# dylandreimerink/mimic

Measured on AMD Instinct MI355X. Metric: Mpkts/s (device-resident, one XDP program over 64-1500B batches), higher is better.
Workload: dtype u64; 1 GPU; cfg2: 1M x 64B xdp_md, 36-slot parse+hash DROP/PASS classifier, per-CPU array E=4 S=8; packets_per_gpu=1048576, vcpus_per_gpu=262144, schedule=interleaved, parallelism=dp1, batches_rotated=8, working_set_bytes=713031680, program_slots=36, engine=spread_own, batches_per_launch=8

## Files before the change

include/mimic_amd.h:

```cpp
#ifndef MIMIC_AMD_H
#define MIMIC_AMD_H

#if !defined(__HIPCC_RTC__)
#include <stddef.h>
#include <stdint.h>
#endif

#ifdef __cplusplus
extern "C" {
#endif

#define MIMIC_ABI_VERSION 4

#define MIMIC_EINVAL (-1)
#define MIMIC_ENOMEM (-2)
#define MIMIC_EDEVICE (-3)
#define MIMIC_ENOTSUP (-4)
#define MIMIC_ENOENT (-5)
#define MIMIC_EFAULT (-6)
#define MIMIC_ECANCELED (-7)
#define MIMIC_EDEADLINE (-8)

enum mimic_status {
    MIMIC_OK = 0,
// ... 4 lines not shown
    MIMIC_ERR_MEM_BOUNDS = 5,
    MIMIC_ERR_MEM_NOT_DATASEC = 6,
    MIMIC_ERR_R10_WRITE = 7,
    MIMIC_ERR_HELPER_MAP_PTR = 8,
    MIMIC_ERR_HELPER_KEY = 9,
    MIMIC_ERR_HELPER_VALUE = 10,
    MIMIC_ERR_HELPER_MAP_OP = 11,
    MIMIC_ERR_HELPER_TAILCALL = 12,
    MIMIC_ERR_HELPER_UNIMPLEMENTED = 13,
    MIMIC_ERR_HELPER_CANT_EMULATE = 14,
    MIMIC_ERR_LDABS = 15,
    MIMIC_PANIC_DIV0 = 16,
    MIMIC_PANIC_SHIFT = 17,
    MIMIC_PANIC_BADREG = 18,
    MIMIC_PANIC_CALLX = 19,
    MIMIC_PANIC_PC = 20,
    MIMIC_PANIC_HELPER_NEG = 21,
    MIMIC_ERR_STEP_LIMIT = 22,
    MIMIC_ERR_CALL_DEPTH = 23,
    MIMIC_ERR_ENGINE_HELPER = 24,
    MIMIC_ERR_NO_CPU = 25,
    MIMIC_ERR_CTX_ACCESS = 26,
    MIMIC_PANIC_SLICE = 27,
    MIMIC_ERR_CTX_LOAD = 28,
    MIMIC_ERR_CANCELED = 29,
    MIMIC_ERR_DEADLINE = 30,
    MIMIC_ERR_ENGINE_STATE = 31
};

#define MIMIC_MAP_HASH 1
#define MIMIC_MAP_ARRAY 2
#define MIMIC_MAP_PROG_ARRAY 3
#define MIMIC_MAP_PERCPU_HASH 5
#define MIMIC_MAP_PERCPU_ARRAY 6

#define MIMIC_MAP_F_DATASEC 1u

#define MIMIC_SCHED_CHUNKED 0
#define MIMIC_SCHED_INTERLEAVED 1
#define MIMIC_SCHED_EXPLICIT 2

typedef struct mimic_vm mimic_vm;

typedef struct {
    int32_t vcpus;
    int32_t stack_frame_size;
    int32_t stack_frame_count;
    int32_t max_tail_calls;
    int32_t device;
    int32_t vcpu_begin;
    int32_t vcpu_count;
    int32_t exec_mode;
} mimic_vm_settings;

#define MIMIC_EXEC_DEFAULT 0
#define MIMIC_EXEC_INTERP 1
#define MIMIC_EXEC_JIT 2
#define MIMIC_EXEC_SPREAD 3
#define MIMIC_EXEC_SPREAD_OWN 4

typedef struct {
    const char *name;
    uint32_t type, key_size, value_size, max_entries, flags;
} mimic_map_spec;

typedef struct {
    uint32_t slot;
    uint32_t map_id;
} mimic_reloc;

typedef struct {
    uint32_t n;
    uint32_t schedule;
    uint8_t *pkt_data;
    const uint64_t *pkt_off;
    const uint32_t *pkt_len;
    const uint32_t *headroom;  uint32_t headroom_all;
    const uint32_t *tailroom;  uint32_t tailroom_all;
    const int32_t *ingress_ifindex; int32_t ingress_all;
    const int32_t *rx_queue_index;  int32_t rxq_all;
    const int32_t *egress_ifindex;  int32_t egress_all;
    const int32_t *cpu;
    uint64_t step_budget;
} mimic_xdp_batch;

typedef struct {
    uint64_t *r0;
    uint8_t *status;
    uint32_t *steps;
    int32_t *err_pc;
} mimic_xdp_results;

int mimic_abi_version(void);
const char *mimic_last_error(const mimic_vm *vm);

int mimic_vm_create(const mimic_vm_settings *settings, mimic_vm **out);
void mimic_vm_destroy(mimic_vm *vm);

int mimic_map_create(mimic_vm *vm, const mimic_map_spec *spec, uint32_t *map_id);
int mimic_map_update(mimic_vm *vm, uint32_t map_id, const void *key, const void *value, uint32_t flags, int32_t cpu);
int mimic_map_update_batch(mimic_vm *vm, uint32_t map_id, const void *keys, const void *values, uint32_t n,
                           uint32_t flags, int32_t cpu, int32_t *rc_out);
int mimic_map_lookup(mimic_vm *vm, uint32_t map_id, const void *key, int32_t cpu, uint32_t *addr_out);
int mimic_map_delete(mimic_vm *vm, uint32_t map_id, const void *key);
int mimic_map_keys(mimic_vm *vm, uint32_t map_id, void *out, size_t cap, uint32_t *n_out);
int mimic_map_entries(mimic_vm *vm, uint32_t map_id, void *keys_out, int32_t *slots_out, size_t cap_entries,
                      uint32_t *n_out);
int mimic_map_read_values(mimic_vm *vm, uint32_t map_id, int32_t cpu, void *out, size_t cap);
int mimic_map_reset(mimic_vm *vm, uint32_t map_id, void *hip_stream);
int mimic_map_read_values_range(mimic_vm *vm, uint32_t map_id, int32_t cpu_begin, int32_t cpu_end, void *out,
                                size_t cap);
int mimic_map_sum_u64(mimic_vm *vm, uint32_t map_id, int32_t cpu_begin, int32_t cpu_end, uint64_t *out, size_t cap);
int mimic_map_share(mimic_vm *vm, uint32_t map_id, mimic_vm *owner, uint32_t owner_map_id);
int mimic_map_addr(mimic_vm *vm, uint32_t map_id, uint32_t *addr_out);

int mimic_program_load(mimic_vm *vm, const char *name, const void *insns, uint32_t n_slots,
                       const mimic_reloc *relocs, uint32_t n_relocs, uint32_t *prog_id);
int mimic_program_addr(mimic_vm *vm, uint32_t prog_id, uint32_t *addr_out);

int mimic_mem_read(mimic_vm *vm, uint32_t addr, void *buf, uint32_t len);
int mimic_mem_load(mimic_vm *vm, uint32_t addr, int32_t size, uint64_t *out);
int mimic_stack_addr(mimic_vm *vm, uint32_t *addr_out);

int mimic_run_xdp(mimic_vm *vm, uint32_t prog_id, const mimic_xdp_batch *batch,
                  const mimic_xdp_results *results, void *hip_stream);
int mimic_run_xdp_many(mimic_vm *vm, uint32_t prog_id, const mimic_xdp_batch *batches,
                       const mimic_xdp_results *results, uint32_t k, void *hip_stream);
#define MIMIC_CTX_XDP 0
#define MIMIC_CTX_SKB 1
#define MIMIC_SKB_CUSTOM_SK 1u
#define MIMIC_SKB_CUSTOM_FLOWKEYS 2u
typedef struct {
    uint32_t flags;
    uint32_t sk_bound_dev_if, sk_family, sk_type, sk_protocol, sk_mark, sk_priority;
    uint32_t sk_src_port, sk_dst_port, sk_state;
    int32_t sk_rx_queue_mapping;
    uint8_t sk_ip_len[4];
    uint8_t sk_ip[4][16];
    uint16_t fk_nhoff, fk_thoff, fk_addr_proto;
    uint8_t fk_is_frag, fk_is_first_frag, fk_is_encap, fk_ip_proto;
    uint16_t fk_n_proto, fk_sport, fk_dport;
    uint32_t fk_flags, fk_flow_label;
} mimic_skb_custom;

typedef struct {
    uint32_t n;
    uint32_t schedule;
    uint8_t *pkt_data;
    const uint64_t *pkt_off;
    const uint32_t *pkt_len;
    uint32_t ifindex;
    int32_t pad;
    const int32_t *cpu;
    uint64_t step_budget;
    const mimic_skb_custom *custom;
    uint32_t *rooms_state;
} mimic_skb_batch;

int mimic_run_skb(mimic_vm *vm, uint32_t prog_id, const mimic_skb_batch *batch,
                  const mimic_xdp_results *results, void *hip_stream);
int mimic_skb_release(mimic_vm *vm);

typedef struct mimic_process mimic_process;
typedef struct {
    uint64_t r[11];
    int32_t pc;
    uint32_t prog_id;
    uint64_t steps;
    int32_t status;
    uint32_t exited;
} mimic_process_regs;
int mimic_process_new(mimic_vm *vm, uint32_t prog_id, const void *packet, uint32_t len, uint32_t headroom,
                      uint32_t tailroom, int32_t ingress_ifindex, int32_t rx_queue_index, int32_t egress_ifindex,
                      mimic_process **out);
int mimic_process_new_skb(mimic_vm *vm, uint32_t prog_id, const void *packet, uint32_t len, uint32_t ifindex,
                          mimic_process **out);
// ... 71 lines not shown
```

mimic_amd/_lib.py:

```python
from __future__ import annotations

import ctypes as C
import os

_HERE = os.path.dirname(os.path.abspath(__file__))
LIB_PATH = os.path.join(_HERE, os.path.basename(os.environ.get("MIMIC_LIB", "libmimic_amd.so")))

ABI_VERSION = 4

STATUS_NAMES = [
    "OK", "ERR_PC_OOB", "ERR_UNSUPPORTED_OP", "ERR_MEM_UNRESOLVED", "ERR_MEM_NOT_VMMEM",
    "ERR_MEM_BOUNDS", "ERR_MEM_NOT_DATASEC", "ERR_R10_WRITE", "ERR_HELPER_MAP_PTR",
    "ERR_HELPER_KEY", "ERR_HELPER_VALUE", "ERR_HELPER_MAP_OP", "ERR_HELPER_TAILCALL",
    "ERR_HELPER_UNIMPLEMENTED", "ERR_HELPER_CANT_EMULATE", "ERR_LDABS", "PANIC_DIV0",
    "PANIC_SHIFT", "PANIC_BADREG", "PANIC_CALLX", "PANIC_PC", "PANIC_HELPER_NEG",
    "ERR_STEP_LIMIT", "ERR_CALL_DEPTH", "ERR_ENGINE_HELPER", "ERR_NO_CPU", "ERR_CTX_ACCESS", "PANIC_SLICE",
    "ERR_CTX_LOAD", "ERR_CANCELED", "ERR_DEADLINE", "ERR_ENGINE_STATE",
]
STATUS = {n: i for i, n in enumerate(STATUS_NAMES)}
ECANCELED, EDEADLINE = -7, -8

SCHED_CHUNKED, SCHED_INTERLEAVED, SCHED_EXPLICIT = 0, 1, 2
MAP_F_DATASEC = 1


class VMSettings(C.Structure):
    _fields_ = [("vcpus", C.c_int32), ("stack_frame_size", C.c_int32), ("stack_frame_count", C.c_int32),
                ("max_tail_calls", C.c_int32), ("device", C.c_int32), ("vcpu_begin", C.c_int32),
                ("vcpu_count", C.c_int32), ("exec_mode", C.c_int32)]


class MapSpecC(C.Structure):
    _fields_ = [("name", C.c_char_p), ("type", C.c_uint32), ("key_size", C.c_uint32),
                ("value_size", C.c_uint32), ("max_entries", C.c_uint32), ("flags", C.c_uint32)]


class ProcessRegs(C.Structure):
    _fields_ = [("r", C.c_uint64 * 11), ("pc", C.c_int32), ("prog_id", C.c_uint32), ("steps", C.c_uint64),
                ("status", C.c_int32), ("exited", C.c_uint32)]


class Reloc(C.Structure):
    _fields_ = [("slot", C.c_uint32), ("map_id", C.c_uint32)]


class XDPBatch(C.Structure):
    _fields_ = [("n", C.c_uint32), ("schedule", C.c_uint32), ("pkt_data", C.c_void_p),
                ("pkt_off", C.c_void_p), ("pkt_len", C.c_void_p),
                ("headroom", C.c_void_p), ("headroom_all", C.c_uint32),
                ("tailroom", C.c_void_p), ("tailroom_all", C.c_uint32),
                ("ingress_ifindex", C.c_void_p), ("ingress_all", C.c_int32),
                ("rx_queue_index", C.c_void_p), ("rxq_all", C.c_int32),
                ("egress_ifindex", C.c_void_p), ("egress_all", C.c_int32),
                ("cpu", C.c_void_p), ("step_budget", C.c_uint64)]


class SKBBatch(C.Structure):
    _fields_ = [("n", C.c_uint32), ("schedule", C.c_uint32), ("pkt_data", C.c_void_p),
                ("pkt_off", C.c_void_p), ("pkt_len", C.c_void_p), ("ifindex", C.c_uint32), ("pad", C.c_int32),
                ("cpu", C.c_void_p), ("step_budget", C.c_uint64), ("custom", C.c_void_p), ("rooms_state", C.c_void_p)]


SKB_CUSTOM_SK, SKB_CUSTOM_FLOWKEYS = 1, 2
try:
    import numpy as _np

    SKB_CUSTOM_DTYPE = _np.dtype([
        ("flags", "<u4"), ("sk_bound_dev_if", "<u4"), ("sk_family", "<u4"), ("sk_type", "<u4"), ("sk_protocol", "<u4"),
        ("sk_mark", "<u4"), ("sk_priority", "<u4"), ("sk_src_port", "<u4"), ("sk_dst_port", "<u4"), ("sk_state", "<u4"),
        ("sk_rx_queue_mapping", "<i4"), ("sk_ip_len", "u1", (4,)), ("sk_ip", "u1", (4, 16)),
        ("fk_nhoff", "<u2"), ("fk_thoff", "<u2"), ("fk_addr_proto", "<u2"), ("fk_is_frag", "u1"),
        ("fk_is_first_frag", "u1"), ("fk_is_encap", "u1"), ("fk_ip_proto", "u1"), ("fk_n_proto", "<u2"),
        ("fk_sport", "<u2"), ("fk_dport", "<u2"), ("fk_flags", "<u4"), ("fk_flow_label", "<u4")])
    assert SKB_CUSTOM_DTYPE.itemsize == 136
except ImportError:
    SKB_CUSTOM_DTYPE = None


CTX_XDP, CTX_SKB = 0, 1


class XDPResults(C.Structure):
    _fields_ = [("r0", C.c_void_p), ("status", C.c_void_p), ("steps", C.c_void_p), ("err_pc", C.c_void_p)]


class XDPHostBatch(C.Structure):
    _fields_ = [("n", C.c_uint32), ("schedule", C.c_uint32), ("pkt_data", C.c_void_p),
                ("pkt_off", C.c_void_p), ("pkt_len", C.c_void_p),
                ("headroom_all", C.c_uint32), ("tailroom_all", C.c_uint32),
                ("ingress_all", C.c_int32), ("rxq_all", C.c_int32), ("egress_all", C.c_int32), ("pad", C.c_int32),
                ("cpu", C.c_void_p), ("step_budget", C.c_uint64), ("pkt_out", C.c_void_p),
                ("r0", C.c_void_p), ("status", C.c_void_p)]


EXPORTS = {
    "mimic_abi_version": (C.c_int, []),
    "mimic_last_error": (C.c_char_p, [C.c_void_p]),
    "mimic_vm_create": (C.c_int, [C.POINTER(VMSettings), C.POINTER(C.c_void_p)]),
    "mimic_vm_destroy": (None, [C.c_void_p]),
    "mimic_map_create": (C.c_int, [C.c_void_p, C.POINTER(MapSpecC), C.POINTER(C.c_uint32)]),
    "mimic_map_update": (C.c_int, [C.c_void_p, C.c_uint32, C.c_void_p, C.c_void_p, C.c_uint32, C.c_int32]),
    "mimic_map_lookup": (C.c_int, [C.c_void_p, C.c_uint32, C.c_void_p, C.c_int32, C.POINTER(C.c_uint32)]),
    "mimic_map_update_batch": (C.c_int, [C.c_void_p, C.c_uint32, C.c_void_p, C.c_void_p, C.c_uint32, C.c_uint32,
                                         C.c_int32, C.c_void_p]),
    "mimic_map_delete": (C.c_int, [C.c_void_p, C.c_uint32, C.c_void_p]),
    "mimic_exec_mode": (C.c_int, [C.c_void_p]),
    "mimic_set_spread": (C.c_int, [C.c_void_p, C.c_int32]),
    "mimic_process_new_skb_ctx": (C.c_int, [C.c_void_p, C.c_uint32, C.c_char_p, C.c_uint32, C.c_uint32, C.c_void_p,
                                            C.POINTER(C.c_void_p)]),
    "mimic_run_xdp_host": (C.c_int, [C.c_void_p, C.c_uint32, C.POINTER(XDPHostBatch), C.c_uint32]),
    "mimic_host_register": (C.c_int, [C.c_void_p, C.c_size_t]),
    "mimic_host_unregister": (C.c_int, [C.c_void_p]),
    "mimic_last_exec": (C.c_int, [C.c_void_p]),
    "mimic_jit_source_for": (C.c_long, [C.POINTER(C.c_void_p), C.POINTER(C.c_uint32), C.c_uint32, C.c_char_p,
                                         C.c_size_t]),
    "mimic_jit_check": (C.c_int, [C.c_char_p, C.c_char_p, C.c_size_t, C.POINTER(C.c_size_t)]),
    "mimic_jit_prebuild": (C.c_int, [C.POINTER(C.c_void_p), C.POINTER(C.c_uint32), C.c_uint32]),
    "mimic_map_keys": (C.c_int, [C.c_void_p, C.c_uint32, C.c_void_p, C.c_size_t, C.POINTER(C.c_uint32)]),
    "mimic_map_entries": (C.c_int, [C.c_void_p, C.c_uint32, C.c_void_p, C.c_void_p, C.c_size_t,
                                    C.POINTER(C.c_uint32)]),
    "mimic_map_read_values": (C.c_int, [C.c_void_p, C.c_uint32, C.c_int32, C.c_void_p, C.c_size_t]),
    "mimic_map_reset": (C.c_int, [C.c_void_p, C.c_uint32, C.c_void_p]),
    "mimic_map_read_values_range": (C.c_int, [C.c_void_p, C.c_uint32, C.c_int32, C.c_int32, C.c_void_p, C.c_size_t]),
    "mimic_map_sum_u64": (C.c_int, [C.c_void_p, C.c_uint32, C.c_int32, C.c_int32, C.c_void_p, C.c_size_t]),
    "mimic_map_addr": (C.c_int, [C.c_void_p, C.c_uint32, C.POINTER(C.c_uint32)]),
    "mimic_program_load": (C.c_int, [C.c_void_p, C.c_char_p, C.c_void_p, C.c_uint32, C.POINTER(Reloc),
                                     C.c_uint32, C.POINTER(C.c_uint32)]),
    "mimic_program_addr": (C.c_int, [C.c_void_p, C.c_uint32, C.POINTER(C.c_uint32)]),
    "mimic_mem_read": (C.c_int, [C.c_void_p, C.c_uint32, C.c_void_p, C.c_uint32]),
    "mimic_mem_load": (C.c_int, [C.c_void_p, C.c_uint32, C.c_int32, C.POINTER(C.c_uint64)]),
    "mimic_stack_addr": (C.c_int, [C.c_void_p, C.POINTER(C.c_uint32)]),
    "mimic_run_xdp": (C.c_int, [C.c_void_p, C.c_uint32, C.POINTER(XDPBatch), C.POINTER(XDPResults), C.c_void_p]),
    "mimic_run_xdp_many": (C.c_int, [C.c_void_p, C.c_uint32, C.POINTER(XDPBatch), C.POINTER(XDPResults), C.c_uint32,
                                     C.c_void_p]),
    "mimic_map_share": (C.c_int, [C.c_void_p, C.c_uint32, C.c_void_p, C.c_uint32]),
    "mimic_run_skb": (C.c_int, [C.c_void_p, C.c_uint32, C.POINTER(SKBBatch), C.POINTER(XDPResults), C.c_void_p]),
    "mimic_skb_release": (C.c_int, [C.c_void_p]),
    "mimic_jit_source_for_ctx": (C.c_long, [C.POINTER(C.c_void_p), C.POINTER(C.c_uint32), C.c_uint32, C.c_int32,
                                             C.c_char_p, C.c_size_t]),
    "mimic_jit_source_vc": (C.c_long, [C.POINTER(C.c_void_p), C.POINTER(C.c_uint32), C.c_uint32, C.c_int32,
                                       C.POINTER(C.c_uint32), C.c_uint32, C.c_char_p, C.c_size_t]),
    "mimic_jit_source_spread": (C.c_long, [C.POINTER(C.c_void_p), C.POINTER(C.c_uint32), C.c_uint32,
                                           C.POINTER(C.c_uint32), C.c_uint32, C.POINTER(C.c_uint32), C.c_uint32,
                                           C.c_uint32, C.POINTER(C.c_int32), C.c_char_p, C.c_size_t]),
    "mimic_jit_prebuild_ctx": (C.c_int, [C.POINTER(C.c_void_p), C.POINTER(C.c_uint32), C.c_uint32, C.c_int32]),
    "mimic_jit_cache_source": (C.c_int, [C.c_char_p]),
    "mimic_process_new": (C.c_int, [C.c_void_p, C.c_uint32, C.c_char_p, C.c_uint32, C.c_uint32, C.c_uint32,
                                    C.c_int32, C.c_int32, C.c_int32, C.POINTER(C.c_void_p)]),
    "mimic_process_new_skb": (C.c_int, [C.c_void_p, C.c_uint32, C.c_char_p, C.c_uint32, C.c_uint32, C.c_void_p]),
    "mimic_process_set_cpu": (C.c_int, [C.c_void_p, C.c_int32]),
    "mimic_process_step": (C.c_int, [C.c_void_p, C.c_uint32, C.c_void_p]),
    "mimic_process_run": (C.c_int, [C.c_void_p, C.c_uint64, C.c_void_p]),
    "mimic_process_packet": (C.c_int, [C.c_void_p, C.c_void_p, C.c_size_t]),
    "mimic_process_free": (None, [C.c_void_p]),
    "mimic_jit_code": (C.c_int, [C.c_char_p, C.c_void_p, C.c_size_t, C.POINTER(C.c_size_t)]),
    "mimic_sync": (C.c_int, [C.c_void_p, C.c_void_p]),
    "mimic_ctx_new": (C.c_int, [C.c_uint64, C.POINTER(C.c_void_p)]),
    "mimic_ctx_cancel": (None, [C.c_void_p]),
    "mimic_ctx_err": (C.c_int, [C.c_void_p]),
    "mimic_ctx_pinned": (C.c_int, [C.c_void_p]),
    "mimic_ctx_free": (None, [C.c_void_p]),
    "mimic_run_xdp_ctx": (C.c_int, [C.c_void_p, C.c_uint32, C.POINTER(XDPBatch), C.POINTER(XDPResults), C.c_void_p,
                                    C.c_void_p, C.c_void_p]),
    "mimic_run_skb_ctx": (C.c_int, [C.c_void_p, C.c_uint32, C.POINTER(SKBBatch), C.POINTER(XDPResults), C.c_void_p,
                                    C.c_void_p, C.c_void_p]),
    "mimic_process_run_ctx": (C.c_int, [C.c_void_p, C.c_uint64, C.c_void_p, C.POINTER(ProcessRegs)]),
    "mimic_process_run_many": (C.c_int, [C.c_void_p, C.c_uint32, C.c_void_p, C.c_void_p, C.POINTER(ProcessRegs)]),
    "mimic_process_free_many": (None, [C.c_void_p, C.c_uint32]),
    "mimic_run_xdp_host_ctx": (C.c_int, [C.c_void_p, C.c_uint32, C.POINTER(XDPHostBatch), C.c_uint32, C.c_void_p]),
    "mimic_run_xdp_host_ctx_pp": (C.c_int, [C.c_void_p, C.c_uint32, C.POINTER(XDPHostBatch), C.c_uint32, C.c_void_p]),
    "mimic_last_steps": (C.c_int, [C.c_void_p, C.POINTER(C.c_uint64)]),
}

_lib = None


def load() -> C.CDLL:
    global _lib
    if _lib is not None:
        return _lib
    if not os.path.exists(LIB_PATH):
        raise ImportError(f"{LIB_PATH} is missing: run __graft_entry__.build() (hipcc --offload-arch=gfx950)")
    try:
        import torch
    except ImportError:
        pass
    lib = C.CDLL(LIB_PATH)
    for name, (res, args) in EXPORTS.items():
        fn = getattr(lib, name)
        fn.restype = res
        fn.argtypes = args
    if lib.mimic_abi_version() != ABI_VERSION:
        raise ImportError("libmimic_amd.so ABI version mismatch")
    _lib = lib
    return lib
```

mimic_amd/csrc/engine.cpp:

```cpp
#include <hip/hip_runtime.h>

#include <algorithm>
#include <atomic>
#include <cstdarg>
#include <cstdlib>
#include <cstdio>
#include <cstring>
#include <map>
#include <string>
#include <chrono>
#include <condition_variable>
#include <memory>
#include <mutex>
#include <thread>
#include <unordered_map>
#include <vector>

#include "../../include/mimic_amd.h"
#include "blkcache.h"
#include "layout.h"
#include "hashmap.h"
#include "jit.h"
#include "skb.h"

// ... 500 lines not shown
    vm->d_segs = nullptr;
    vm->d_maps = nullptr;
    HIP_OK(vm, hipMalloc(&vm->d_insns, all.size() * sizeof(DInsn)));
    HIP_OK(vm, hipMalloc(&vm->d_progs, dp.size() * sizeof(DProg)));
    HIP_OK(vm, hipMalloc(&vm->d_segs, sg.size() * sizeof(Seg)));
    HIP_OK(vm, hipMalloc(&vm->d_maps, dm.size() * sizeof(DMap)));
    HIP_OK(vm, hipMemcpy(vm->d_insns, all.data(), all.size() * sizeof(DInsn), hipMemcpyHostToDevice));
    HIP_OK(vm, hipMemcpy(vm->d_progs, dp.data(), dp.size() * sizeof(DProg), hipMemcpyHostToDevice));
    HIP_OK(vm, hipMemcpy(vm->d_segs, sg.data(), sg.size() * sizeof(Seg), hipMemcpyHostToDevice));
    HIP_OK(vm, hipMemcpy(vm->d_maps, dm.data(), dm.size() * sizeof(DMap), hipMemcpyHostToDevice));
    vm->tables_dirty = false;
    return 0;
}

struct HostRef {
    int kind;
    uint64_t dev_off;
    uint32_t off, limit;
};

static HostRef host_resolve(const mimic_vm *vm, uint32_t a) {
    HostRef R{0, 0, 0, 0};
    for (const Seg &g : vm->segs) {
        if (a < g.lo || a > g.hi) continue;
        uint32_t off = a - g.lo;
        switch (g.kind) {
        case SEG_PLAIN: R = {1, g.dev_off, off, g.size}; break;
        case SEG_ARRAY_OBJ: R = {g.datasec ? 1 : 3, g.dev_off, off, g.size}; break;
        case SEG_MAP_OBJ: case SEG_PROG: R = {2, 0, 0, 0}; break;
        case SEG_PERCPU_ARRAY: {
            uint32_t c = off / g.period, r = off - c * g.period;
            uint64_t base = g.dev_off + (uint64_t)c * g.dev_stride;
            if (r <= 8) R = {g.datasec ? 1 : 3, base, r, g.size};
            else R = {1, base, r - 9, g.size};
            break;
        }
        case SEG_PERCPU_VALUES: {
            uint32_t c = off / g.period, r = off - c * g.period;
            R = {1, g.dev_off + (uint64_t)c * g.dev_stride, r, g.size};
            break;
        }
        }
        return R;
    }
    return R;
}

static int decode_program(const uint8_t *raw, uint32_t n_slots, std::vector<DInsn> &out, std::string *err) {
    out.assign(n_slots, DInsn{0, 0, 0});
    for (uint32_t i = 0; i < n_slots; i++) {
        const uint8_t *b = raw + 8ull * i;
        uint32_t op = b[0], dst = b[1] & 0xf, src = b[1] >> 4;
        uint16_t off = (uint16_t)(b[2] | (b[3] << 8));
        int32_t imm;
        memcpy(&imm, b + 4, 4);
        DInsn d{};
        d.w = op | (dst << 8) | (src << 12) | ((uint32_t)off << 16);
        d.k = (uint64_t)(int64_t)imm;
        if (op == 0x18) {
            if (i + 1 >= n_slots) {
                *err = "64bit immediate is missing second half";
                return -1;
            }
            const uint8_t *c = b + 8;
            if (c[0] | c[1] | c[2] | c[3]) {
                *err = "64bit immediate has non-zero fields";
                return -1;
            }
            uint32_t hi;
            memcpy(&hi, c + 4, 4);
            d.k = ((uint64_t)hi << 32) | (uint32_t)imm;
            out[i] = d;
            out[++i] = DInsn{0, 0, 0};
            continue;
        }
        out[i] = d;
    }
    return 0;
}

extern "C" {

int mimic_abi_version(void) { return MIMIC_ABI_VERSION; }

const char *mimic_last_error(const mimic_vm *vm) { return vm ? vm->err.c_str() : "null vm"; }

int mimic_vm_create(const mimic_vm_settings *settings, mimic_vm **out) {
    if (!settings || !out) return MIMIC_EINVAL;
    if (settings->vcpus <= 0) return MIMIC_EINVAL;
    mimic_vm *vm = new mimic_vm();
    vm->s = *settings;
    if (vm->s.stack_frame_size <= 0) vm->s.stack_frame_size = 256;
    if (vm->s.stack_frame_count <= 0) vm->s.stack_frame_count = 8;
    if (vm->s.vcpu_count <= 0) {
        vm->s.vcpu_begin = 0;
        vm->s.vcpu_count = vm->s.vcpus;
    }
    if (vm->s.vcpu_begin < 0 || vm->s.vcpu_begin + vm->s.vcpu_count > vm->s.vcpus) {
        delete vm;
        return MIMIC_EINVAL;
    }
    if (stack_size(vm) % 8 != 0 || stack_size(vm) > (1u << 20)) {
        delete vm;
        return MIMIC_EINVAL;
    }
    vm->exec_mode = settings->exec_mode;
    if (vm->exec_mode == MIMIC_EXEC_DEFAULT) {
        const char *e = getenv("MIMIC_EXEC");
        vm->exec_mode = (e && !strcmp(e, "interp")) ? MIMIC_EXEC_INTERP : MIMIC_EXEC_JIT;
    }
    if (const char *pj = getenv("MIMIC_PROC_JIT")) vm->proc_jit_after = *pj ? atoll(pj) : 32;
    if (vm->exec_mode != MIMIC_EXEC_INTERP && vm->exec_mode != MIMIC_EXEC_JIT) {
        delete vm;
        return MIMIC_EINVAL;
    }
    if (hipSetDevice(vm->s.device) != hipSuccess || hipStreamCreateWithFlags(&vm->stream, hipStreamNonBlocking) != hipSuccess) {
        delete vm;
        return MIMIC_EDEVICE;
    }
    *out = vm;
    return 0;
}

void mimic_vm_destroy(mimic_vm *vm) {
    if (!vm) return;
    hipSetDevice(vm->s.device);
    hipDeviceSynchronize();
    for (auto &m : vm->maps) {
        if (!m.share) continue;
        auto &mem = m.share->members;
        if (!mem.empty() && mem[0].vm == vm) m.share->owner_gone = true;
        for (size_t k = 0; k < mem.size(); k++)
            if (mem[k].vm == vm) {
                if (k == 0) hipDeviceSynchronize();
                mem.erase(mem.begin() + (long)k);
                break;
            }
        m.share.reset();
    }
    vm->blk.drain([](Blk &b) {
        hipFree(b.dev);
        if (b.host) hipHostFree(b.host);
    });
    hipFree(vm->arena);
    hipFree(vm->d_insns);
    hipFree(vm->d_progs);
    hipFree(vm->d_segs);
    hipFree(vm->d_maps);
    hipFree(vm->priv);
    hipFree(vm->d_sched_start);
    hipFree(vm->d_sched_pkts);
    hipFree(vm->d_lane_steps);
    hipFree(vm->d_spread_bad);
    hipFree(vm->d_spread_part);
    hipFree(vm->d_cancel_pp);
    hipFree(vm->d_defer);
    hipFree(vm->d_defer_any);
    hipFree(vm->d_kp);
    if (vm->h_kp) hipHostFree(vm->h_kp);
    for (auto &sl : vm->slot) {
        hipFree(sl.buf);
        hipFree(sl.off);
        hipFree(sl.len);
        hipFree(sl.r0);
        hipFree(sl.st);
        for (hipEvent_t e : {sl.e_in, sl.e_k, sl.e_out})
// ... 775 lines not shown
    g.lo = p.addr;
    g.hi = p.addr + 8;
    g.kind = SEG_PROG;
    g.id = (uint32_t)vm->progs.size();
    vm->segs.push_back(g);
    vm->progs.push_back(std::move(p));
    vm->tables_dirty = true;
    *prog_id = g.id;
    return 0;
}

int mimic_program_addr(mimic_vm *vm, uint32_t prog_id, uint32_t *addr_out) {
    if (!vm || prog_id >= vm->progs.size()) return MIMIC_EINVAL;
    *addr_out = vm->progs[prog_id].addr;
    return 0;
}

int mimic_stack_addr(mimic_vm *vm, uint32_t *addr_out) {
    if (!vm) return MIMIC_EINVAL;
    *addr_out = vm->next_addr;
    return 0;
}

int mimic_mem_read(mimic_vm *vm, uint32_t addr, void *buf, uint32_t len) {
    if (!vm) return MIMIC_EINVAL;
    hipSetDevice(vm->s.device);
    HostRef R = host_resolve(vm, addr);
    if (R.kind == 0) return fail(vm, MIMIC_EFAULT, "memory controller can't resolve address 0x%x", addr);
    if (R.kind == 2) return fail(vm, MIMIC_EFAULT, "not vm memory 0x%x", addr);
    if (R.kind == 3) return fail(vm, MIMIC_EFAULT, "Can't access non-data-section array map directly");
    if ((uint64_t)R.off + len > R.limit) return fail(vm, MIMIC_EFAULT, "out of bounds");
    if (int rc = flush_host(vm)) return rc;
    if (vm->last_stream) HIP_OK(vm, hipStreamSynchronize(vm->last_stream));
    HIP_OK(vm, hipMemcpy(buf, vm->arena + R.dev_off + R.off, len, hipMemcpyDeviceToHost));
    return 0;
}

int mimic_mem_load(mimic_vm *vm, uint32_t addr, int32_t size, uint64_t *out) {
    if (size != 1 && size != 2 && size != 4 && size != 8) return MIMIC_EINVAL;
    uint64_t v = 0;
    int rc = mimic_mem_read(vm, addr, &v, (uint32_t)size);
    if (rc) return rc;
    *out = v;
    return 0;
}

struct SkbRun {
    uint32_t ifindex;
    const mimic_skb_custom *custom;
    const uint64_t *pre_drv = nullptr, *pre_prefix = nullptr, *pre_base = nullptr;
    uint32_t *rooms_state = nullptr;
};
struct StepRun {
    StepState *state;
    uint8_t *priv;
    uint64_t priv_bytes;
    uint64_t budget;
    SkbRec *skb_rec = nullptr;
    const uint64_t *skb_prefix = nullptr, *skb_base = nullptr;
    const mimic_skb_custom *skb_custom = nullptr;
    uint32_t gen = 0;
    const uint8_t *img = nullptr;
    uint8_t *img_dst = nullptr;
    uint32_t img_n = 0;
    bool jit = false;
    int32_t cpu = 0;
};

struct CtxRun {
    mimic_ctx *all;
    mimic_ctx *const *per_packet;
    const uint32_t *const *dev_pp = nullptr;
};
struct ManyRun {
    const mimic_xdp_batch *b;
    const mimic_xdp_results *r;
    uint32_t k;
    bool used;
};
static int run_xdp_impl(mimic_vm *vm, uint32_t prog_id, const mimic_xdp_batch *b, const mimic_xdp_results *res,
                        hipStream_t st_in, uint64_t shift, const SkbRun *skb = nullptr, const StepRun *step = nullptr,
                        const CtxRun *cx = nullptr, ManyRun *mr = nullptr);

int mimic_run_xdp(mimic_vm *vm, uint32_t prog_id, const mimic_xdp_batch *b, const mimic_xdp_results *res,
                  void *hip_stream) {
    return run_xdp_impl(vm, prog_id, b, res, (hipStream_t)hip_stream, 0);
}

int mimic_run_xdp_many(mimic_vm *vm, uint32_t prog_id, const mimic_xdp_batch *b, const mimic_xdp_results *res, uint32_t k,
                       void *hip_stream) {
    if (!vm || (k && (!b || !res))) return MIMIC_EINVAL;
    hipStream_t st = (hipStream_t)hip_stream;
    auto same = [&](const mimic_xdp_batch &x, const mimic_xdp_batch &y) {
        return x.n == y.n && x.schedule == y.schedule && x.schedule != MIMIC_SCHED_EXPLICIT && !x.headroom && !y.headroom &&
               !x.tailroom && !y.tailroom && !x.ingress_ifindex && !y.ingress_ifindex && !x.rx_queue_index &&
               !y.rx_queue_index && !x.egress_ifindex && !y.egress_ifindex && x.headroom_all == y.headroom_all &&
               x.tailroom_all == y.tailroom_all && x.ingress_all == y.ingress_all && x.rxq_all == y.rxq_all &&
               x.egress_all == y.egress_all && x.step_budget == y.step_budget;
    };
    for (uint32_t a = 0; a < k;) {
        uint32_t e = a + 1;
        while (e < k && e - a < MIMIC_MANY_MAX && same(b[a], b[e])) e++;
        ManyRun mr{b + a, res + a, e - a, false};
        int rc = run_xdp_impl(vm, prog_id, b + a, res + a, st, 0, nullptr, nullptr, nullptr, e - a > 1 ? &mr : nullptr);
        if (rc) return rc;
        if (!mr.used)
            for (uint32_t q = a + 1; q < e; q++)
                if ((rc = run_xdp_impl(vm, prog_id, b + q, res + q, st, 0))) return rc;
        a = e;
    }
    return 0;
}

int mimic_run_xdp_ctx(mimic_vm *vm, uint32_t prog_id, const mimic_xdp_batch *b, const mimic_xdp_results *res,
                      void *hip_stream, mimic_ctx *ctx, mimic_ctx *const *ctx_per_packet) {
    const CtxRun cx{ctx, ctx_per_packet};
    return run_xdp_impl(vm, prog_id, b, res, (hipStream_t)hip_stream, 0, nullptr, nullptr, &cx);
}

static int run_skb_impl(mimic_vm *vm, uint32_t prog_id, const mimic_skb_batch *sb, const mimic_xdp_results *res,
                        void *hip_stream, const CtxRun *cx);

int mimic_run_skb(mimic_vm *vm, uint32_t prog_id, const mimic_skb_batch *sb, const mimic_xdp_results *res,
                  void *hip_stream) {
    return run_skb_impl(vm, prog_id, sb, res, hip_stream, nullptr);
}

int mimic_run_skb_ctx(mimic_vm *vm, uint32_t prog_id, const mimic_skb_batch *sb, const mimic_xdp_results *res,
                      void *hip_stream, mimic_ctx *ctx, mimic_ctx *const *ctx_per_packet) {
    const CtxRun cx{ctx, ctx_per_packet};
    return run_skb_impl(vm, prog_id, sb, res, hip_stream, &cx);
}

static int run_skb_impl(mimic_vm *vm, uint32_t prog_id, const mimic_skb_batch *sb, const mimic_xdp_results *res,
                        void *hip_stream, const CtxRun *cx) {
    if (!vm || !sb || !res) return MIMIC_EINVAL;
    mimic_xdp_batch b{};
    b.n = sb->n;
    b.schedule = sb->schedule;
    b.pkt_data = sb->pkt_data;
    b.pkt_off = sb->pkt_off;
    b.pkt_len = sb->pkt_len;
    b.cpu = sb->cpu;
    b.step_budget = sb->step_budget;
    SkbRun r{sb->ifindex, sb->custom};
    r.rooms_state = sb->rooms_state;
    return run_xdp_impl(vm, prog_id, &b, res, (hipStream_t)hip_stream, 0, &r, nullptr, cx);
}

int mimic_skb_release(mimic_vm *vm) {
    if (!vm) return MIMIC_EINVAL;
    hipSetDevice(vm->s.device);
    if (vm->skb_stream) {
        if (!vm->skb_ev) HIP_OK(vm, hipEventCreateWithFlags(&vm->skb_ev, hipEventDisableTiming));
        HIP_OK(vm, hipEventRecord(vm->skb_ev, vm->skb_stream));
        vm->skb_stream = nullptr;
        vm->skb_release_pending = true;
    }
    vm->skb_leaked = false;
    return 0;
}

static int skb_settle(mimic_vm *vm) {
    if (vm->skb_release_pending) HIP_OK(vm, hipEventSynchronize(vm->skb_ev));
    vm->skb_release_pending = false;
    return 0;
}

struct SkbInto {
    SkbRec *rec;
    uint64_t *prefix;
};
static int skb_ensure(mimic_vm *vm, uint32_t n, hipStream_t st);
static int skb_prepare(mimic_vm *vm, const mimic_xdp_batch *b, hipStream_t st, const SkbInto *into = nullptr,
                       uint32_t *rooms_state = nullptr) {
// ... 105 lines not shown

static int spread_build_own(mimic_vm *vm) {
    if (vm->spread_own_state) return 0;
    vm->spread_own_state = -1;
    SpreadReq req;
    req.own = true;
    for (size_t s = 0; s < vm->h_all.size(); s++) {
        const DInsn &x = vm->h_all[s];
        const uint32_t mh = AUX_MAPHINT(x.aux);
        if (AUX_H(x.aux) != H_LDIMM || !mh || mh > vm->maps.size()) continue;
        const HostMap &hm = vm->maps[mh - 1];
        const DMap dm = to_dmap(hm);
        if (hm.family != FAM_PERCPU_ARRAY || (dm.dev_off & 7) || (dm.dev_stride & 7)) continue;
        req.slot_map[(uint32_t)s] = mh - 1;
        req.shape[mh - 1] = {hm.max_entries * hm.value_size, hm.value_size};
    }
    if (req.slot_map.empty()) return 0;
    uint32_t row = 0;
    for (auto &kv : req.shape) row = std::max(row, kv.second.first);
    if (!row) return 0;
    req.lds_rows = std::min<uint32_t>(256u, 32768u / row);
    if (req.lds_rows < 2) return 0;
    JitInfo info{};
    const std::string src = mimic_jit_source(vm->h_dp, vm->h_all, CTX_XDP, &info, nullptr, false, &req);
    if (!info.spread || !info.spread_own) return 0;
    std::string log;
    if (mimic_jit_compile(vm->s.device, src, &vm->jit_fn_spread_own, &log))
        return fail(vm, MIMIC_EDEVICE, "JIT build failed (owned spread kernel): %s", log.c_str());
    vm->jit_info_spread_own = info;
    vm->spread_own_rows = req.lds_rows;
    vm->spread_own_state = 1;
    return 0;
}

static int priv_ensure(mimic_vm *vm, uint32_t q_per_lane, uint32_t lanes, hipStream_t st) {
    const uint32_t stride = std::max(lanes, vm->priv_lanes);
    const uint64_t need = (uint64_t)q_per_lane * stride * 8;
    if (vm->priv && need <= vm->priv_bytes) return 0;
    hipStreamSynchronize(st);
    hipFree(vm->priv);
    vm->priv = nullptr;
    HIP_OK(vm, hipMalloc(&vm->priv, std::max<uint64_t>(need, 8)));
    vm->priv_bytes = std::max<uint64_t>(need, 8);
    vm->priv_lanes = stride;
    return 0;
}

static int spread_check(mimic_vm *vm) {
    if (vm->comb_used) {
        for (const HostMap &m : vm->maps) {
            if (!is_hash(m)) continue;
            uint64_t rb, fo, co;
            ht_offsets(m, &rb, &fo, &co);
            uint32_t f = 0;
            HIP_OK(vm, hipMemcpy(&f, vm->arena + m.ht_dev_off + co + offsetof(HashCtl, comb_fault), 4, hipMemcpyDeviceToHost));
            if (f) return fail(vm, MIMIC_EDEVICE, "map '%s': a block combiner or chunk refill of freelist reservations gave up (engine fault)",
                               m.name.c_str());
        }
    }
    if (!vm->spread_used || !vm->d_spread_bad) return 0;
    uint32_t f = 0;
    HIP_OK(vm, hipMemcpy(&f, vm->d_spread_bad, 4, hipMemcpyDeviceToHost));
    if (f) return fail(vm, MIMIC_EDEVICE, "a spread launch reached per-CPU map memory outside a fused increment");
    return 0;
}

static std::vector<std::pair<uint32_t, uint32_t>> vc_slots_of(const mimic_vm *vm) {
    std::vector<std::pair<uint32_t, uint32_t>> vc;
    for (size_t s = 0; s < vm->h_all.size(); s++) {
        const DInsn &x = vm->h_all[s];
        const uint32_t mh = AUX_MAPHINT(x.aux);
        if (AUX_H(x.aux) != H_LDIMM || !mh || mh > vm->maps.size()) continue;
        const HostMap &hm = vm->maps[mh - 1];
        if (vc_row_ok(hm.family, hm.max_entries, hm.value_size)) vc.push_back({(uint32_t)s, hm.max_entries * hm.value_size});
    }
    return vc;
}

static int run_xdp_impl(mimic_vm *vm, uint32_t prog_id, const mimic_xdp_batch *b, const mimic_xdp_results *res,
                        hipStream_t st_in, uint64_t first_index, const SkbRun *skb, const StepRun *step,
                        const CtxRun *cx, ManyRun *mr) {
    if (!vm || !b || !res) return MIMIC_EINVAL;
    if (prog_id >= vm->progs.size()) return fail(vm, MIMIC_EINVAL, "no program with id '%u' is loaded", prog_id);
    if (b->n > 0 && (!b->pkt_data || !b->pkt_off || !b->pkt_len)) return fail(vm, MIMIC_EINVAL, "missing packet arrays");
    if (cx && cx->all && cx->per_packet) return fail(vm, MIMIC_EINVAL, "one context for the batch or one per packet, not both");
    if (cx && cx->all && !cx->all->pinned) return fail(vm, MIMIC_EDEVICE, "the context was made without a device");
    if (cx && cx->per_packet)
        for (uint32_t i = 0; i < b->n; i++)
            if (cx->per_packet[i] && !cx->per_packet[i]->pinned)
                return fail(vm, MIMIC_EDEVICE, "packet %u: the context was made without a device", i);
    if (!skb) {
        const int rc = skb_settle(vm);
        if (rc) return rc;
    }
    if (!skb && vm->skb_leaked)
        return fail(vm, MIMIC_ENOTSUP, "xdp_md batches after sk_buff batches are not supported (mimic_skb_release first)");
    const uint32_t ctx = skb ? CTX_SKB : CTX_XDP;
    hipSetDevice(vm->s.device);
    int rc = upload_tables(vm);
    if (!rc) rc = flush_host(vm);
    if (rc) return rc;
    hipStream_t st = st_in ? st_in : vm->stream;
    const uint32_t cpu_lanes = step ? 1u : (uint32_t)vm->s.vcpu_count;
    const bool proc_jit = step && step->jit;
    bool extra = false;
    if (!step && b->schedule == MIMIC_SCHED_EXPLICIT && b->cpu)
        for (uint32_t i = 0; i < b->n && !extra; i++) extra = b->cpu[i] == -1 || b->cpu[i] == vm->s.vcpus;
    const uint32_t lanes = cpu_lanes + (extra ? 2u : 0u);
    const uint32_t S = stack_size(vm);
    const PrivPlan pp = priv_plan(vm);
    const uint32_t xdp_q = pp.xdp_q, frame_q = pp.frame_q, key_q = pp.key_q, q_per_lane = pp.q_per_lane;
    const uint32_t plan = (lanes + 255) & ~255u;
    if (step) {
        if (step->priv_bytes < (uint64_t)q_per_lane * 8) return fail(vm, MIMIC_EINVAL, "process private memory too small");
    } else {
        rc = priv_ensure(vm, q_per_lane, plan, st);
        if (rc) return rc;
    }
    if (lanes > vm->lane_steps_cap) {
        hipStreamSynchronize(st);
        hipFree(vm->d_lane_steps);
        vm->d_lane_steps = nullptr;
        HIP_OK(vm, hipMalloc(&vm->d_lane_steps, (uint64_t)plan * sizeof(uint64_t)));
        vm->lane_steps_cap = plan;
    }
    KParams kp{};
    kp.insns = vm->d_insns;
    kp.progs = vm->d_progs;
    kp.segs = vm->d_segs;
    kp.maps = vm->d_maps;
    kp.arena = vm->arena;
    kp.nprogs = (uint32_t)vm->progs.size();
    kp.nsegs = (uint32_t)vm->segs.size();
    kp.nmaps = (uint32_t)vm->maps.size();
    kp.entry_prog = prog_id;
    kp.static_next = vm->next_addr;
    kp.stack_size = S;
    kp.frame_size = (uint32_t)vm->s.stack_frame_size;
    uint32_t shift = 3;
    while (S > 512 && ((S - 512 + (1u << shift) - 1) >> shift) > 64) shift++;
    kp.chunk_shift = shift;
    kp.max_tail_calls = (uint32_t)std::max(0, vm->s.max_tail_calls);
    kp.total_vcpus = (uint32_t)vm->s.vcpus;
    kp.vcpu_begin = proc_jit ? (uint32_t)step->cpu : (uint32_t)vm->s.vcpu_begin;
    kp.lanes = lanes;
    kp.cpu_lanes = cpu_lanes;
    kp.priv_lanes = step ? 1u : vm->priv_lanes;
    kp.priv = step ? step->priv : vm->priv;
    kp.priv_xdp_q = xdp_q;
    kp.priv_frame_q = frame_q;
    kp.priv_key_q = key_q;
    kp.budget = step ? step->budget : (b->step_budget ? b->step_budget : MIMIC_DEFAULT_BUDGET);
    kp.step = step ? step->state : nullptr;
    kp.step_gen = step ? step->gen : 0u;
    if (step) {
        kp.step_img = step->img;
        kp.step_dst = step->img_dst;
        kp.step_img_n = step->img_n;
        kp.step_ins_n = (uint32_t)std::min<size_t>(vm->h_all.size(), 2048);
    }
    kp.n = b->n;
    kp.sched = b->schedule;
    kp.pkt_data = b->pkt_data;
    kp.pkt_off = b->pkt_off;
    kp.pkt_len = b->pkt_len;
    kp.headroom_arr = b->headroom;
    kp.tailroom_arr = b->tailroom;
    kp.ingress_arr = b->ingress_ifindex;
    kp.rxq_arr = b->rx_queue_index;
    kp.egress_arr = b->egress_ifindex;
    kp.headroom = b->headroom_all;
    kp.tailroom = b->tailroom_all;
    kp.ingress = b->ingress_all;
    kp.rxq = b->rxq_all;
    kp.egress = b->egress_all;
    kp.r0 = res->r0;
    kp.status = res->status;
    kp.steps = res->steps;
    kp.err_pc = res->err_pc;
    kp.lane_steps = vm->d_lane_steps;
    if (cx && cx->all) {
        kp.cancel = cx->all->dword;
        kp.cancel_any = 1;
    } else if (cx && cx->dev_pp && b->n) {
        kp.cancel_pp = cx->dev_pp;
        kp.cancel_any = 1;
    } else if (cx && cx->per_packet && b->n) {
        std::vector<const uint32_t *> w(b->n);
        bool any = false;
        for (uint32_t i = 0; i < b->n; i++) {
            w[i] = cx->per_packet[i] ? cx->per_packet[i]->dword : nullptr;
            any |= w[i] != nullptr;
        }
        if (any) {
            if (vm->cancel_pp_stream) hipStreamSynchronize(vm->cancel_pp_stream);
            hipStreamSynchronize(st);
            vm->cancel_pp_stream = st;
            if (b->n > vm->cancel_pp_cap) {
                hipFree(vm->d_cancel_pp);
                vm->d_cancel_pp = nullptr;
                HIP_OK(vm, hipMalloc(&vm->d_cancel_pp, (size_t)b->n * sizeof(void *)));
                vm->cancel_pp_cap = b->n;
            }
            HIP_OK(vm, hipMemcpy(vm->d_cancel_pp, w.data(), (size_t)b->n * sizeof(void *), hipMemcpyHostToDevice));
            kp.cancel_pp = vm->d_cancel_pp;
            kp.cancel_any = 1;
        }
    }
    switch (b->schedule) {
    case MIMIC_SCHED_CHUNKED:
        kp.per_lane = lanes ? (uint32_t)(((uint64_t)b->n + lanes - 1) / lanes) : 0;
        break;
    case MIMIC_SCHED_INTERLEAVED:
        kp.sched_shift = lanes ? (uint32_t)(first_index % lanes) : 0;
        kp.per_lane = lanes ? (uint32_t)(((uint64_t)b->n + kp.sched_shift + lanes - 1) / lanes) : 0;
        break;
    case MIMIC_SCHED_EXPLICIT: {
        if (!b->cpu && b->n) return fail(vm, MIMIC_EINVAL, "explicit schedule needs cpu[]");
        std::vector<uint32_t> start(lanes + 1, 0), pk(b->n);
        std::vector<uint32_t> lane_of(b->n);
        for (uint32_t i = 0; i < b->n; i++) {
            const int32_t id = b->cpu[i];
            int64_t c = (int64_t)id - vm->s.vcpu_begin;
            if (id == -1) c = cpu_lanes;
            else if (id == vm->s.vcpus) c = cpu_lanes + 1;
            else if (c < 0 || c >= (int64_t)cpu_lanes)
                return fail(vm, MIMIC_EINVAL, "packet %u: cpu %d not on this engine", i, id);
            lane_of[i] = (uint32_t)c;
            start[c + 1]++;
        }
        uint32_t mx = 0;
        for (uint32_t c = 0; c < lanes; c++) {
            mx = std::max(mx, start[c + 1]);
            start[c + 1] += start[c];
        }
        std::vector<uint32_t> fill(start.begin(), start.end() - 1);
        for (uint32_t i = 0; i < b->n; i++) pk[fill[lane_of[i]]++] = i;
        hipStreamSynchronize(st);
        if (start.size() > vm->sched_cap_start) {
            hipFree(vm->d_sched_start);
            vm->d_sched_start = nullptr;
            HIP_OK(vm, hipMalloc(&vm->d_sched_start, start.size() * 4));
            vm->sched_cap_start = start.size();
        }
        if (pk.size() > vm->sched_cap_pkts || !vm->d_sched_pkts) {
            hipFree(vm->d_sched_pkts);
            vm->d_sched_pkts = nullptr;
            HIP_OK(vm, hipMalloc(&vm->d_sched_pkts, std::max<size_t>(pk.size(), 1) * 4));
// ... 116 lines not shown
            }
            kp.spread_part = vm->d_spread_part;
        }
    }
    if (skb && step && step->skb_rec) {
        kp.ctx_kind = CTX_SKB;
        kp.skb_ifindex = skb->ifindex;
        kp.skb_rec = step->skb_rec;
        kp.skb_prefix = step->skb_prefix;
        kp.skb_base = step->skb_base;
        kp.skb_custom = step->skb_custom;
    } else if (skb && skb->pre_drv) {
        rc = skb_ensure(vm, b->n, st);
        if (rc) return rc;
        kp.ctx_kind = CTX_SKB;
        kp.skb_ifindex = skb->ifindex;
        kp.skb_rec = vm->d_skb_rec;
        kp.skb_drv = skb->pre_drv;
        kp.skb_prefix = skb->pre_prefix;
        kp.skb_base = skb->pre_base;
        kp.skb_custom = skb->custom;
        vm->skb_stream = st;
    } else if (skb) {
        rc = skb_prepare(vm, b, st, nullptr, skb->rooms_state);
        if (rc) return rc;
        kp.skb_rooms_state = skb->rooms_state;
        kp.ctx_kind = CTX_SKB;
        kp.skb_ifindex = skb->ifindex;
        kp.skb_rec = vm->d_skb_rec;
        kp.skb_drv = vm->d_skb_drv;
        kp.skb_prefix = vm->d_skb_prefix;
        kp.skb_base = vm->d_skb_state + 1;
        kp.skb_custom = skb->custom;
    }
    kp.hash_pop_only = vm->prog_deletes ? 0u : 1u;
    kp.hash_ro = (vm->prog_deletes || vm->prog_updates) ? 0u : 1u;
    for (auto &m : vm->maps) {
        if (!is_hash(m)) continue;
        if (m.share) {
            if ((rc = share_check(vm, m))) return rc;
            for (auto &mb : m.share->members) {
                mimic_vm *o = (mimic_vm *)mb.vm;
                if (o != vm && o->host_dirty && (rc = flush_host(o))) return fail(vm, rc, "shared map: %s", o->err.c_str());
            }
            share_stale(m);
        }
        const DMap dm = to_dmap(m);
        if (vm->prog_deletes && m.pop_dirty) {
            if (mimic_launch_hash_normalize(vm->arena, &dm, st))
                return fail(vm, MIMIC_EDEVICE, "launch: %s", hipGetErrorString(hipGetLastError()));
            m.pop_dirty = false;
        }
        if (!vm->prog_deletes) m.pop_dirty = true;
        if (vm->prog_deletes) m.may_tomb = true;
        if (m.mir && (vm->prog_updates || vm->prog_deletes || m.may_tomb)) m.mir->valid = false;
        if (!m.may_tomb) continue;
        if (mimic_launch_hash_rebuild(vm->arena, &dm, 0, st))
            return fail(vm, MIMIC_EDEVICE, "launch: %s", hipGetErrorString(hipGetLastError()));
    }
    vm->last_exec = jit ? (own ? MIMIC_EXEC_SPREAD_OWN : spread ? MIMIC_EXEC_SPREAD : MIMIC_EXEC_JIT) : MIMIC_EXEC_INTERP;
    if (jit && ji.defer) {
        if (lanes > vm->defer_cap || !vm->d_defer_any) {
            hipStreamSynchronize(st);
            hipFree(vm->d_defer);
            vm->d_defer = nullptr;
            HIP_OK(vm, hipMalloc(&vm->d_defer, (uint64_t)plan * sizeof(DeferRec)));
            HIP_OK(vm, hipMemset(vm->d_defer, 0, (uint64_t)plan * sizeof(DeferRec)));
            vm->defer_cap = plan;
            if (!vm->d_defer_any) {
                HIP_OK(vm, hipMalloc(&vm->d_defer_any, 64));
                HIP_OK(vm, hipMemset(vm->d_defer_any, 0, 64));
            }
        }
        if (++vm->defer_epoch == 0) vm->defer_epoch = 1;
        kp.defer = vm->d_defer;
        kp.defer_any = vm->d_defer_any;
        kp.defer_epoch = vm->defer_epoch;
    }
    if (jit && ji.hash_combine) vm->comb_used = true;
    if (mr) {
        mr->used = jit && own && !ji.defer && mr->k >= 1 && mr->k <= MIMIC_MANY_MAX;
        if (mr->used) {
            kp.many_n = mr->k;
            for (uint32_t q = 0; q < mr->k; q++)
                kp.many[q] = BatchRef{mr->b[q].pkt_data, mr->b[q].pkt_off, mr->b[q].pkt_len, mr->r[q].r0, mr->r[q].status,
                                      mr->r[q].steps, mr->r[q].err_pc, 0};
        }
    }
    if (jit) {
        if (mimic_jit_launch(jfn, &kp, st))
            return fail(vm, MIMIC_EDEVICE, "launch: %s", hipGetErrorString(hipGetLastError()));
        if (ji.defer && mimic_launch_xdp_resume(&kp, st))
            return fail(vm, MIMIC_EDEVICE, "launch: %s", hipGetErrorString(hipGetLastError()));
    } else if (step) {
        if (mimic_launch_xdp(&kp, nullptr, st))
            return fail(vm, MIMIC_EDEVICE, "launch: %s", hipGetErrorString(hipGetLastError()));
    } else {
        const KParams *dkp = nullptr;
        const int slot = kp_slot(vm, kp, st, &dkp);
        if (slot < 0) return slot;
        if (mimic_launch_xdp(&kp, dkp, st))
            return fail(vm, MIMIC_EDEVICE, "launch: %s", hipGetErrorString(hipGetLastError()));
        HIP_OK(vm, hipEventRecord(vm->kp_ev[slot], st));
        vm->kp_used[slot] = true;
    }
    if (jit && ji.hash_chunk) {
        for (const HostMap &m : vm->maps) {
            if (!m.chunk) continue;
            const DMap dm = to_dmap(m);
            if (mimic_launch_hash_compact(vm->arena, &dm, st))
                return fail(vm, MIMIC_EDEVICE, "launch: %s", hipGetErrorString(hipGetLastError()));
        }
    }
    if (jit && kp.spread_part) {
        const DMap dm = to_dmap(vm->maps[ji.spread_map]);
        if (mimic_launch_spread_reduce(kp.spread_part, kp.lanes / 256u, kp.cpu_lanes, ji.spread_roww, ji.spread_n,
                                       vm->arena + dm.dev_off + (uint64_t)kp.vcpu_begin * dm.dev_stride, dm.dev_stride, st))
            return fail(vm, MIMIC_EDEVICE, "launch: %s", hipGetErrorString(hipGetLastError()));
    }
    if (kp.cancel_any) {
        auto mark = [&](mimic_ctx *c) -> int {
            std::lock_guard<std::mutex> lk(c->mu);
            std::vector<hipEvent_t> keep;
            for (hipEvent_t e : c->uses) {
                if (hipEventQuery(e) == hipSuccess) hipEventDestroy(e);
                else keep.push_back(e);
            }
            c->uses.swap(keep);
            hipEvent_t ev = nullptr;
            HIP_OK(vm, hipEventCreateWithFlags(&ev, hipEventDisableTiming));
            HIP_OK(vm, hipEventRecord(ev, st));
            c->uses.push_back(ev);
            return 0;
        };
        if (cx->all) {
            if ((rc = mark(cx->all))) return rc;
        } else {
            std::vector<mimic_ctx *> u;
            for (uint32_t i = 0; i < b->n; i++)
                if (cx->per_packet[i]) u.push_back(cx->per_packet[i]);
            std::sort(u.begin(), u.end());
            u.erase(std::unique(u.begin(), u.end()), u.end());
            for (mimic_ctx *c : u)
                if ((rc = mark(c))) return rc;
        }
    }
    vm->last_lanes = run_lanes;
    vm->last_stream = st;
    return 0;
}

}

namespace {
constexpr size_t PD_LEN = 8, PD_SKB = 64;
constexpr size_t PD_PKT = (PD_SKB + sizeof(SkbRec) + 24 + sizeof(mimic_skb_custom) + 63) & ~(size_t)63;
constexpr size_t PH_RES = (sizeof(StepState) + 63) & ~(size_t)63;
constexpr size_t PH_R0 = PH_RES, PH_ST = PH_RES + 8, PH_STEPS = PH_RES + 16, PH_EPC = PH_RES + 20, PH_WORD = PH_RES + 24;
constexpr size_t PH_IMG = PH_RES + 64;
}

struct mimic_process {
    mimic_vm *vm = nullptr;
    uint32_t prog = 0;
    uint32_t H = 0, T = 0, len = 0;
    int32_t ingress = 0, rxq = 0, egress = 0;
    uint8_t *d_pkt = nullptr;
    uint8_t *d_skbmem = nullptr;
    StepState *hs = nullptr;
// ... 888 lines not shown
```

mimic_amd/csrc/interp.hip:

```cpp
#include <hip/hip_runtime.h>
#include <stdint.h>
#include <algorithm>
#include <cstdlib>

#include "runtime.h"
static_assert(sizeof(Lane) <= sizeof(((StepState *)0)->lane), "StepState::lane too small");
static __device__ void step_save(const KParams &kp, const Lane &L, const uint64_t *RB, int st, int32_t pc, uint32_t steps,
                                 uint32_t prog) {
    StepState *S = kp.step;
    for (int q = 0; q < 11; q++) S->r[q] = RB[q * 64];
    __builtin_memcpy(S->lane, &L, sizeof(Lane));
    S->pc = pc;
    S->prog = prog;
    S->steps = steps;
    S->status = st;
    S->started = 1;
    S->finished = st != MIMIC_ERR_STEP_LIMIT;
}

#define WAVES_PER_BLOCK 4

static __device__ __noinline__ void step_warm(const KParams &kp, uint32_t t, uint32_t nt) {
    const DProg last = kp.progs[kp.nprogs - 1];
    const uint64_t spans[5][2] = {{(uint64_t)(uintptr_t)kp.insns, (uint64_t)(last.base + last.n) * sizeof(DInsn)},
                                  {(uint64_t)(uintptr_t)kp.segs, (uint64_t)kp.nsegs * sizeof(Seg)},
                                  {(uint64_t)(uintptr_t)kp.maps, (uint64_t)kp.nmaps * sizeof(DMap)},
                                  {(uint64_t)(uintptr_t)kp.progs, (uint64_t)kp.nprogs * sizeof(DProg)},
                                  {(uint64_t)(uintptr_t)kp.pkt_data, 512}};
    uint32_t n = 0;
    for (int k = 0; k < 5; k++) {
        const uint64_t lines = (spans[k][1] + 63) / 64;
        for (uint64_t q = t; q < lines && q < 4096; q += nt) n += *(const volatile uint32_t *)(spans[k][0] + q * 64);
    }
    if (t == 0) n += *(const volatile uint32_t *)kp.pkt_off + *(const volatile uint32_t *)kp.pkt_len;
    (void)n;
}
#define NREGS 11
#define KEY_DONE 0xffffffffu

enum { MODE_BATCH = 0, MODE_STEP = 1, MODE_RESUME = 2 };
template <int MODE>
static __device__ __forceinline__ void xdp_body(const KParams *__restrict__ kpp, uint32_t goff = 0) {
    const KParams &kp = *kpp;
    StepState *const STP = MODE == MODE_STEP ? kp.step : nullptr;
    __shared__ uint64_t sreg[WAVES_PER_BLOCK][NREGS][64];
    uint64_t *const RB = &sreg[threadIdx.x >> 6][0][threadIdx.x & 63];
#define REG(r) RB[(r) * 64]

    const uint32_t g = goff + blockIdx.x * blockDim.x + threadIdx.x;
    const DeferRec *DR = nullptr;
    uint32_t j0 = 0;
    if (MODE == MODE_RESUME) {
        if (*kp.defer_any != kp.defer_epoch) return;
        if (g < kp.lanes && kp.defer[g].flag == kp.defer_epoch) {
            DR = kp.defer + g;
            j0 = DR->j;
        }
        if (__ballot(DR != nullptr) == 0) return;
    }
    const bool lane_valid = g < kp.lanes && (MODE != MODE_RESUME || DR);
    extern __shared__ DInsn step_ins_[];
    if (MODE == MODE_STEP) {
        if (kp.step_img) {
            typedef uint32_t u32x4 __attribute__((ext_vector_type(4)));
            const uint32_t nq = kp.step_img_n >> 4;
            for (uint32_t q = threadIdx.x; q < nq; q += blockDim.x)
                ((u32x4 *)kp.step_dst)[q] = ((const u32x4 *)kp.step_img)[q];
            for (uint32_t b = (nq << 4) + threadIdx.x; b < kp.step_img_n; b += blockDim.x) kp.step_dst[b] = kp.step_img[b];
        }
        for (uint32_t q = threadIdx.x; q < kp.step_ins_n; q += blockDim.x) step_ins_[q] = kp.insns[q];
        __syncthreads();
        if (threadIdx.x >= 64) step_warm(kp, threadIdx.x - 64, blockDim.x - 64);
    }
    Lane L;
    L.lane = g;
    L.cpu = STP ? STP->cpu : lane_cpu(kp, g);

    uint32_t ex_begin = 0, ex_count = 0;
    if (lane_valid && kp.sched == SCHED_EXPLICIT) {
        ex_begin = kp.sched_start[g];
        ex_count = kp.sched_start[g + 1] - ex_begin;
    }
    uint64_t lane_steps = MODE == MODE_RESUME && DR ? DR->lane_steps : 0;
    const DProg entry = cget(kp.progs, kp.entry_prog);
    const uint32_t P = kp.static_next + kp.stack_size + 1;

    for (uint32_t j = 0; j < kp.per_lane; j++) {
        uint32_t i = 0xffffffffu;
        if (lane_valid && (MODE != MODE_RESUME || j >= j0)) {
            if (kp.sched == SCHED_CHUNKED) {
                uint64_t ii = (uint64_t)g * kp.per_lane + j;
                if (ii < kp.n) i = (uint32_t)ii;
            } else if (kp.sched == SCHED_INTERLEAVED) {
                uint64_t ii = (uint64_t)j * kp.lanes + (g >= kp.sched_shift ? g - kp.sched_shift : g + kp.lanes - kp.sched_shift);
                if (ii < kp.n) i = (uint32_t)ii;
            } else if (j < ex_count) {
                i = kp.sched_pkts[ex_begin + j];
            }
        }

#pragma unroll
        for (int q = 0; q < NREGS; q++) REG(q) = 0;
        uint32_t pn = entry.n, pbase = entry.base;
        uint32_t cur_prog = kp.entry_prog;
        uint32_t key = KEY_DONE;
        uint32_t steps = 0;
        L.sm0 = 0;
        L.sm1 = 0;
        L.xdp_dirty = 0;
        L.t_n = 0;
        L.t_lo = 0;
        L.t_ptr = nullptr;
        L.nframes = 0;
        L.tailcalls = 0;
        L.M = 0;
        L.pkt = nullptr;
        L.rec = nullptr;
        L.pa = P;
        L.ka = 0;
#define TERM(st_, epc_)                                                \
        do {                                                           \
            if (kp.r0) kp.r0[i] = REG(0);                              \
            if (kp.status) kp.status[i] = (uint8_t)(st_);              \
            if (kp.steps) kp.steps[i] = steps;                         \
            if (kp.err_pc) kp.err_pc[i] = (int32_t)(epc_);             \
            lane_steps += steps;                                       \
            key = KEY_DONE;                                            \
            if (STP) step_save(kp, L, RB, (st_), (epc_), steps, cur_prog); \
        } while (0)
        bool resumed = false, foreign = false;
        if (i != 0xffffffffu && STP && STP->gen != kp.step_gen) {
            foreign = true;
            if (kp.r0) kp.r0[i] = 0;
            if (kp.status) kp.status[i] = (uint8_t)MIMIC_ERR_ENGINE_STATE;
            if (kp.steps) kp.steps[i] = 0;
            if (kp.err_pc) kp.err_pc[i] = -1;
        } else if (i != 0xffffffffu && STP && STP->started) {
            const StepState *S = STP;
#pragma unroll
            for (int q = 0; q < NREGS; q++) REG(q) = S->r[q];
            __builtin_memcpy(&L, S->lane, sizeof(Lane));
            L.cpu = S->cpu;
            steps = S->steps;
            cur_prog = S->prog;
            const DProg cp = kp.progs[cur_prog];
            pn = cp.n;
            pbase = cp.base;
            resumed = true;
            if (S->pc < 0) {
                steps++;
                TERM(MIMIC_PANIC_PC, S->pc);
            } else {
                key = pbase + (uint32_t)S->pc;
            }
        }
        const bool resume_here = MODE == MODE_RESUME && i != 0xffffffffu && j == j0;
        if (resumed || foreign) {
        } else if (i != 0xffffffffu && kp.ctx_kind == CTX_SKB) {
            uint64_t r1 = 0;
            const int ls = skb_load(kp, L, i, r1, resume_here);
            REG(10) = kp.static_next + kp.frame_size;
            if (ls) {
                TERM(ls, -1);
            } else {
                REG(1) = r1;
                key = pbase;
                if (pn == 0) {
                    steps = 1;
                    TERM(MIMIC_ERR_PC_OOB, 0);
                }
            }
        } else if (i != 0xffffffffu) {
            const uint32_t H = kp.headroom_arr ? kp.headroom_arr[i] : kp.headroom;
            const uint32_t T = kp.tailroom_arr ? kp.tailroom_arr[i] : kp.tailroom;
            const uint32_t len = kp.pkt_len[i];
            L.pkt = kp.pkt_data + kp.pkt_off[i];
            L.M = H + len + T;
            if (!resume_here) {
                for (uint32_t b = 0; b < H; b++) L.pkt[b] = 0;
                for (uint32_t b = 0; b < T; b++) L.pkt[H + len + b] = 0;
            }
            L.data = P + H;
            L.data_end = P + H + len;
            L.ingress = (uint32_t)(kp.ingress_arr ? kp.ingress_arr[i] : kp.ingress);
            L.rxq = (uint32_t)(kp.rxq_arr ? kp.rxq_arr[i] : kp.rxq);
            L.egress = (uint32_t)(kp.egress_arr ? kp.egress_arr[i] : kp.egress);
            REG(1) = P + L.M + 1;
            REG(10) = kp.static_next + kp.frame_size;
            key = pbase;
            if (pn == 0) {
                steps = 1;
                TERM(MIMIC_ERR_PC_OOB, 0);
            }
        }

        if (resume_here) {
#pragma unroll
            for (int q = 0; q < NREGS; q++) REG(q) = DR->r[q];
            L.sm0 = DR->sm0;
            L.sm1 = DR->sm1;
            L.xdp_dirty = DR->xdp_dirty;
            L.nframes = DR->nframes;
            L.tailcalls = DR->tailcalls;
            steps = DR->steps;
            cur_prog = DR->prog;
            const DProg cp = kp.progs[cur_prog];
            pn = cp.n;
            pbase = cp.base;
            key = pbase + (uint32_t)DR->pc;
            resumed = true;
        }

        if (MODE != MODE_STEP && kp.cancel_any && !resumed && key != KEY_DONE) {
            const uint32_t cz = ctx_done(kp, i);
            if (cz) TERM(MIMIC_ERR_CANCELED - 1 + (int)cz, (int32_t)(key - pbase));
        }
        uint64_t wsteps = resumed ? steps : 0;
        uint32_t cand = KEY_DONE;
        for (;;) {
            if (MODE != MODE_STEP && kp.cancel_any && (wsteps & 4095u) == 4095u && key != KEY_DONE) {
                const uint32_t cz = ctx_done(kp, i);
                if (cz) TERM(MIMIC_ERR_CANCELED - 1 + (int)cz, (int32_t)(key - pbase));
            }
            uint32_t kw;
            uint64_t act;
            if (MODE == MODE_STEP) {
                kw = (uint32_t)__builtin_amdgcn_readfirstlane((int)key);
                if (kw == KEY_DONE) break;
                act = 1;
            } else {
                const uint64_t live = __ballot(key != KEY_DONE);
                if (live == 0) break;
                if (cand != KEY_DONE && (__ballot(key != cand) & live) == 0) kw = cand;
                else kw = wave_min(key);
                kw = (uint32_t)__builtin_amdgcn_readfirstlane((int)kw);
                act = __ballot(key == kw);
            }
            const DInsn in = MODE == MODE_STEP && kw < kp.step_ins_n ? step_ins_[kw] : cget(kp.insns, kw);
            const uint64_t wbefore = wsteps++;
            if (key == kw) {
                const uint32_t pc = kw - pbase;
                if (wbefore >= kp.budget && (uint64_t)steps == kp.budget) {
                    TERM(MIMIC_ERR_STEP_LIMIT, pc);
                } else {
                    steps++;
                    const uint32_t aux = in.aux;
                    const uint32_t op = in.w & 0xff;
                    const uint32_t dst = (in.w >> 8) & 0xf, src = (in.w >> 12) & 0xf;
                    const int32_t off = (int16_t)(in.w >> 16);
                    const uint64_t k = in.k;
                    int st = 0;
                    int jmp = 0;
                    uint32_t nk = 0;
                    switch (AUX_H(aux)) {
                    case H_NOP:
                        break;
                    case H_ALU64: {
                        const uint64_t d = REG(dst);
                        const uint64_t x = (aux & AUX_X) ? REG(src) : k;
// ... 549 lines not shown
```

mimic_amd/csrc/jit.cpp:

```cpp
#include <hip/hip_runtime.h>
#include <hip/hiprtc.h>

#include <algorithm>
#include <cinttypes>
#include <cstdarg>
#include <cstdio>
#include <cstring>
#include <cstdlib>
#include <unistd.h>
#include <map>
#include <mutex>
#include <set>
#include <string>
#include <vector>

#include "../../include/mimic_amd.h"
#include "layout.h"
#include "jit.h"

namespace {

#include "jit_headers.inc"

struct Emitter {
// ... 213 lines not shown
            hash_combine = combine_knob && writes && !deletes && cold_inline && fast_paths;
            if (hash_combine) E.line("#define MIMIC_HASH_COMBINE 1");
            hash_chunk = hash_combine && !proc && hchunk_knob > 0;
            if (hash_chunk) E.line("#define MIMIC_HASH_CHUNK 1\n#define MIMIC_HCHUNK %uu", (uint32_t)hchunk_knob);
        }
        E.line("#include \"runtime.h\"");
        if (spread_on) {
            E.line("#define SPREAD_MAP %uu        // the per-CPU array the fused increments go to", spread_map);
            E.line("#define SPREAD_N %uu          // counter width (bytes)", spread_n);
            E.line("#define SPREAD_ROWW %uu       // counters per vCPU row (E * S / N)", spread_row / spread_n);
            E.line("#define SPREAD_ROWS %uu       // LDS table rows (0: agent-scope atomics into the map)", spread_req->lds_rows);
            E.line("#define SPREAD_PPB %uu        // packets per block", spread_req->ppb);
            E.line("typedef %s spread_t;", spread_n == 8 ? "unsigned long long" : "uint32_t");
            E.line("#if SPREAD_ROWS");
            E.line("#define spread_add(k_) __hip_atomic_fetch_add(&sacc_[srow_ * SPREAD_ROWW + (uint32_t)(ga_ - L.t_lo) / SPREAD_N], (spread_t)(k_), __ATOMIC_RELAXED, __HIP_MEMORY_SCOPE_WORKGROUP)");
            E.line("#else");
            E.line("#define spread_add(k_) __hip_atomic_fetch_add((GAS spread_t *)(L.t_ptr + (uint32_t)(ga_ - L.t_lo)), (spread_t)(k_), __ATOMIC_RELAXED, __HIP_MEMORY_SCOPE_AGENT)");
            E.line("#endif");
        }
        if (proc) {
            E.line("#define PGID_ kp.entry_prog");
            E.line("#define TERM(s_, pc_) do { st_ = (int)(s_); epc_ = (int32_t)(pc_); pg_ = PGID_; goto L_term; } while (0)");
        } else {
            E.line("#define TERM(s_, pc_) do { st_ = (int)(s_); epc_ = (int32_t)(pc_); goto L_term; } while (0)");
        }
        E.line("#define SPILL() do { sp_.L = L; sp_.r[0] = r0; sp_.r[1] = r1; sp_.r[2] = r2; sp_.r[3] = r3; sp_.r[4] = r4; "
               "sp_.r[5] = r5; sp_.r[6] = r6; } while (0)");
        E.line("#define FILL() do { r0 = sp_.r[0]; r1 = sp_.r[1]; r2 = sp_.r[2]; r3 = sp_.r[3]; r4 = sp_.r[4]; r5 = sp_.r[5]; "
               "L.sm0 = sp_.L.sm0; L.sm1 = sp_.L.sm1; L.xdp_dirty = sp_.L.xdp_dirty; L.t_lo = sp_.L.t_lo; L.t_n = sp_.L.t_n; "
               "L.t_ptr = sp_.L.t_ptr; } while (0)");
        E.line("#define COLD_CALL(call_, pc_) do { VC_FLUSH(); SPILL(); call_; FILL(); if (sp_.st) TERM(sp_.st, pc_); } while (0)");
        E.line("#define DFR(pc_, prog_) do { dr_->pc = (int32_t)(pc_); dr_->prog = (prog_); dr_->steps = steps - 1u; goto L_defer; } while (0)");
        if (vc_on && vc_lds)
            E.line("#define VC_FLUSH() do { if (vcd_) { lvc_writeback(vcp_, vcb_, lvt_); vcd_ = 0u; } vcv_ = 0u; } while (0)");
        else if (vc_on)
            E.line("#define VC_FLUSH() do { if (vcd_) { vc_writeback(vcp_, vcb_, vc0_, vc1_, vc2_, vc3_); vcd_ = 0u; } vcv_ = 0u; } while (0)");
        else
            E.line("#define VC_FLUSH() do { } while (0)");
        const int wv = proc ? 0 : waves > 0 ? waves : (cold_inline ? 4 : 0);
        E.line("extern \"C\" __global__ __launch_bounds__(256) %svoid mimic_jit_kernel(const KParams kp_arg_) {",
               wv > 0 ? ("__attribute__((amdgpu_waves_per_eu(" + std::to_string(wv) + "))) ").c_str() : "");
        E.line("  (void)kp_arg_;   // the first (only) kernel argument: at offset 0 of the kernarg segment");
        E.line("  const KParams __attribute__((address_space(4))) *kp4_ = (const KParams __attribute__((address_space(4))) *)__builtin_amdgcn_kernarg_segment_ptr();");
        E.line("  asm volatile(\"\" : \"+s\"(kp4_));");
        E.line("  const KParams *kpp = (const KParams *)kp4_;");
        E.line("  const KParams &kp = *kpp;");
        E.line("  const uint32_t g = blockIdx.x * blockDim.x + threadIdx.x;");
        if (hash_chunk) E.line("  h_chunk_init(%s);   // (its waves: those the early return below keeps)", spread_on ? "0xffffffffu" : "kp.lanes");
        if (hash_combine) E.line("  h_comb_init();   // before any thread of the block can leave");
        if (!spread_on) E.line("  if (g >= kp.lanes) return;");
        skb_lds = ctx == CTX_SKB && fast_paths && skb_fields && skb_lds_knob;
        if (skb_lds) E.line("  __shared__ uint64_t srec_[%uu * 256u];", kSrecQ);
        E.line("  Lane L;");
        E.line("  Spill sp_;");
        if (census) {
            E.line("  uint32_t coldn_ = 0;");
            E.line("#define COLD_CALL_K(k_, call_, pc_) do { coldn_ += 1u << (k_); COLD_CALL(call_, pc_); } while (0)");
        }
        E.line("  L.lane = g;");
        if (spread_own) {
            E.line("  const uint32_t oP_ = kp.per_lane, oQ_ = kp.own_q, oS_ = oP_ / oQ_, oR_ = 256u / oS_;");
            E.line("  const uint32_t orow_ = threadIdx.x %% oR_, oj_ = threadIdx.x / oR_, olane_ = blockIdx.x * oR_ + orow_;");
            E.line("  const uint32_t osh_ = olane_ >= kp.sched_shift ? olane_ - kp.sched_shift : olane_ + kp.cpu_lanes - kp.sched_shift;");
            E.line("#define OWN_IDX_I(k_) ((oj_ < oS_ && olane_ < kp.cpu_lanes && (uint64_t)(oj_ + (k_) * oS_) * kp.cpu_lanes + osh_ < kp.n) ? (uint32_t)((uint64_t)(oj_ + (k_) * oS_) * kp.cpu_lanes + osh_) : NO_PKT)");
            E.line("#define OWN_IDX_C(k_) ((threadIdx.x + 256u * (k_) < oR_ * oP_ && (uint64_t)blockIdx.x * oR_ * oP_ + threadIdx.x + 256u * (k_) < kp.n) ? (uint32_t)((uint64_t)blockIdx.x * oR_ * oP_ + threadIdx.x + 256u * (k_)) : NO_PKT)");
            E.line("#define OWN_IDX(k_) (kp.sched == SCHED_CHUNKED ? OWN_IDX_C(k_) : OWN_IDX_I(k_))");
            E.line("  const uint32_t oi_ = OWN_IDX(0u);");
            E.line("  const bool ochk_ = kp.sched == SCHED_CHUNKED;");
            E.line("  const uint64_t ostr64_ = ochk_ ? 256ull : (uint64_t)oS_ * kp.cpu_lanes;");
            E.line("  const uint64_t oend_ = (uint64_t)blockIdx.x * oR_ * oP_ + (uint32_t)(oR_ * oP_);");
            E.line("  uint32_t ofl_ = __builtin_amdgcn_readfirstlane((kp.headroom_arr || kp.tailroom_arr || kp.ingress_arr || kp.rxq_arr || kp.egress_arr ? 1u : 0u) | (kp.headroom | kp.tailroom ? 2u : 0u));");
            E.line("  uint32_t ocpu_ = kp.vcpu_begin + olane_, oep_ = kp.entry_prog, or10_ = kp.static_next + kp.frame_size;");
            E.line("  uint32_t ostr_ = ostr64_ < 0xffffffffull ? (uint32_t)ostr64_ : 0xffffffffu;");
            E.line("  uint32_t olim_ = ochk_ && oend_ < kp.n ? (uint32_t)oend_ : kp.n;");
            E.line("  asm volatile(\"\" : \"+s\"(ostr_), \"+s\"(olim_), \"+s\"(ofl_), \"+s\"(oep_), \"+s\"(or10_));");
            E.line("  asm volatile(\"\" : \"+v\"(ocpu_));");
            E.line("  uint32_t oin_ = (uint32_t)kp.ingress, orx_ = (uint32_t)kp.rxq, oeg_ = (uint32_t)kp.egress;");
            E.line("  asm volatile(\"\" : \"+s\"(oin_), \"+s\"(orx_), \"+s\"(oeg_));");
            E.line("%s", kOwnHoist);
            E.line("  const DMap SM_ = cget(kp.maps, SPREAD_MAP);");
            E.line("  __shared__ spread_t sacc_[SPREAD_ROWS * SPREAD_ROWW];");
            E.line("  for (uint32_t w_ = threadIdx.x; w_ < SPREAD_ROWS * SPREAD_ROWW; w_ += 256u) sacc_[w_] = 0;");
            E.line("  __shared__ BatchRef obr_[MIMIC_MANY_MAX];");
            E.line("  if (threadIdx.x < (kp.many_n ? kp.many_n : 1u)) obr_[threadIdx.x] = kp.many_n ? cget(kp.many, threadIdx.x) : BatchRef{kp.pkt_data, kp.pkt_off, kp.pkt_len, kp.r0, kp.status, kp.steps, kp.err_pc, 0};");
            E.line("  __syncthreads();");
            E.line("  uint32_t srow_ = orow_, sbase_ = 0;");
            E.line("  const bool ofw_ = threadIdx.x < oR_ * SPREAD_ROWW && blockIdx.x * oR_ + threadIdx.x / SPREAD_ROWW < kp.cpu_lanes;");
            E.line("  GAS spread_t *const ofd_ = (GAS spread_t *)(kp.arena + SM_.dev_off + (size_t)(kp.vcpu_begin + blockIdx.x * oR_ + threadIdx.x / SPREAD_ROWW) * SM_.dev_stride) + threadIdx.x %% SPREAD_ROWW;");
            E.line("  const spread_t ofv_ = ofw_ ? *ofd_ : (spread_t)0;");
        } else if (spread_on) {
            E.line("  const uint32_t blo_ = blockIdx.x * SPREAD_PPB, bhi_ = blo_ + SPREAD_PPB < kp.n ? blo_ + SPREAD_PPB : kp.n;");
            E.line("  const uint32_t lam0_ = spread_lane(kp, blo_);");
            E.line("  const DMap SM_ = cget(kp.maps, SPREAD_MAP);");
            E.line("#if SPREAD_ROWS");
            E.line("  __shared__ spread_t sacc_[SPREAD_ROWS * SPREAD_ROWW];");
            E.line("  for (uint32_t w_ = threadIdx.x; w_ < SPREAD_ROWS * SPREAD_ROWW; w_ += 256u) sacc_[w_] = 0;");
            E.line("  __syncthreads();");
            E.line("#endif");
            E.line("  uint32_t srow_ = 0, sbase_ = 0;");
            E.line("  const uint32_t lstep_ = 256u %% kp.cpu_lanes;");
            E.line("  uint32_t lam_ = spread_lane(kp, blo_ + threadIdx.x);");
        } else {
            E.line("  L.cpu = lane_cpu(kp, g);");
        }
        if (vc_on) {
            if (vc_lds) {
                E.line("  __shared__ uint32_t lvc_[(%uu / 4u + 2u) * 256u];", vc_rb);
                E.line("  uint32_t *const lvt_ = lvc_ + threadIdx.x;");
                E.line("  constexpr uint32_t vcb_ = %uu;   // the row's bytes", vc_rb);
                E.line("  uint32_t vcv_ = 0u, vcd_ = 0u, vclo_ = 0u; uint8_t *vcp_ = nullptr;");
                E.line("  { const uint32_t mh_ = AUX_MAPHINT(cget(kp.insns, %uu).aux);", vc_slot);
                E.line("    if (mh_) lvc_open(kp, cget(kp.maps, mh_ - 1u), L.cpu, vcb_, vcp_, vclo_, vcv_, lvt_); }");
            } else {
                E.line("  uint64_t vc0_ = 0, vc1_ = 0, vc2_ = 0, vc3_ = 0; uint32_t vcv_ = 0u, vcd_ = 0u, vclo_ = 0u, vcb_ = 0u; uint8_t *vcp_ = nullptr;");
                E.line("  { const uint32_t mh_ = AUX_MAPHINT(cget(kp.insns, %uu).aux);", vc_slot);
                E.line("    if (mh_) vc_open(kp, cget(kp.maps, mh_ - 1u), L.cpu, vcp_, vclo_, vcb_, vcv_, vc0_, vc1_, vc2_, vc3_); }");
            }
        }
        E.line("  uint32_t ex_begin = 0, ex_count = 0;");
        E.line("  if (kp.sched == SCHED_EXPLICIT) { ex_begin = *gp(kp.sched_start + g); ex_count = *gp(kp.sched_start + g + 1) - ex_begin; }");
        E.line("  uint64_t lane_steps = 0;");
        E.line("  const uint32_t P = kp.static_next + kp.stack_size + 1;");
        if (ctx == CTX_SKB) E.line("  const uint32_t SK_ = P;   // the sk_buff entry (skb.h)");
        E.line("  uint32_t ga_ = 0;   // the address of the current memory access");
        if (ret_dispatch && any_local) E.line("  uint32_t ret_ = 0;   // the slot a popped frame returns to (R<p>_)");
        for (auto &f : fwd_store) E.line("  uint32_t fwd%u_%u_ = 0;   // value of the stack store at P%u slot %u", f.first, f.second, f.first, f.second);
        for (auto &u : spec_use)
            E.line("  %s sp%u_%u_ = 0;   // packet load of P%u slot %u, issued early", u.second == 8 ? "uint64_t" : "uint32_t",
                   u.first.first, u.first.second, u.first.first, u.first.second);
        if (!spec_use.empty()) E.line("  uint32_t spv_ = 1;   // 0 once a store through R10 left the stack: early values void");
        const bool pf = ctx == CTX_XDP && prefetch;
        if (!spec_use.empty() && !spread_on) analyze_xpf();
        lpf_on = pf && xpf.on && lpf_knob && !xpf_knob && !spread_on && !vc_lds && !lds_stack_on && !defer_mode &&
                 !hash_combine && lpf_safe();
        if (!lpf_on && !xpf_knob) xpf.on = false;
        if (spread_own) {
            if (pf) E.line("  uint64_t noff_ = 0, poff_ = 0; uint32_t nlen_ = 0, plen_ = 0;");
            E.line("  const uint32_t nb_ = kp.many_n ? kp.many_n : 1u;");
            E.line("  bool bpre_ = false;   // this batch's first descriptor came with the previous batch's last packet");
            E.line("  for (uint32_t bt_ = 0; bt_ < nb_; bt_++) {");
            E.line("  const BatchRef br_ = kp.many_n ? cget(kp.many, bt_) : BatchRef{kp.pkt_data, kp.pkt_off, kp.pkt_len, kp.r0, kp.status, kp.steps, kp.err_pc, 0};");
        }
        if (lpf_on) {
            const uint32_t D = kLpfD, XW = xpf.words;
            E.line("  // lane prefetch: packets 0..%u of the lane, descriptors + P%u slot %u window (data + %u, %u words)", D - 1,
                   xpf.prog, xpf.hp, (uint32_t)xpf.off, XW);
            E.line("  __shared__ uint64_t lpfo_[%uu * 256u];", D);
            E.line("  __shared__ uint32_t lpfl_[%uu * 256u];", D);
            E.line("  __shared__ uint64_t lpfw_[%uu * 256u];", D * XW);
            E.line("  uint32_t lpf_n_ = 0u, xc_ok_ = 0u;");
            E.line("  if (kp.entry_prog == %uu && !kp.headroom_arr && !kp.tailroom_arr && kp.headroom == 0u && kp.tailroom == 0u) {", xpf.prog);
            for (uint32_t d = 0; d < D; d++) {
                E.line("    const uint32_t lx%u_ = pkt_index(kp, g, %uu, ex_begin, ex_count);", d, d);
                E.line("    uint64_t lo%u_ = 0; uint32_t ll%u_ = 0;", d, d);
                E.line("    if (lx%u_ != NO_PKT) { lo%u_ = *gp(kp.pkt_off + lx%u_); ll%u_ = *gp(kp.pkt_len + lx%u_); }", d, d, d, d, d);
            }
            for (uint32_t d = 0; d < D; d++) {
                for (uint32_t q = 0; q < XW; q++) E.line("    uint64_t lw%u_%u_ = 0;", d, q);
                E.line("    const bool lk%u_ = lx%u_ != NO_PKT && %uu <= ll%u_;", d, d, (uint32_t)xpf.off + 8 * XW, d);
                E.line("    if (lk%u_) {", d);
                E.line("      const uint8_t *xp_ = kp.pkt_data + lo%u_ + %uu;", d, (uint32_t)xpf.off);
                for (uint32_t q = 0; q < XW; q++) E.line("      lw%u_%u_ = ld_n(xp_ + %uu, 8u);", d, q, 8 * q);
                E.line("    }");
            }
            for (uint32_t d = 0; d < D; d++) {
                E.line("    lpfo_[%uu * 256u + threadIdx.x] = lo%u_;", d, d);
                E.line("    lpfl_[%uu * 256u + threadIdx.x] = ll%u_ | (lk%u_ ? 0x80000000u : 0u);", d, d, d);
                for (uint32_t q = 0; q < XW; q++) E.line("    lpfw_[%uu * 256u + threadIdx.x] = lw%u_%u_;", d * XW + q, d, q);
            }
            E.line("    lpf_n_ = lx0_ == NO_PKT ? 0u : lx1_ == NO_PKT ? 1u : lx2_ == NO_PKT ? 2u : lx3_ == NO_PKT ? 3u : 4u;");
            E.line("  }");
            static_assert(kLpfD == 4, "the lpf_n_ line above");
        } else if (pf && xpf.on) {
            E.line("  const bool xpf_on_ = kp.entry_prog == %uu && !kp.headroom_arr;   // P%u slot %u window, data + %u, %u words",
                   xpf.prog, xpf.prog, xpf.hp, (uint32_t)xpf.off, xpf.words);
            E.line("  uint64_t noff_ = 0, noff2_ = 0; uint32_t nlen_ = 0, nlen2_ = 0, nidx_ = NO_PKT, nidx2_ = NO_PKT, xn_ok_ = 0u, xc_ok_ = 0u;");
            for (uint32_t q = 0; q < xpf.words; q++) E.line("  uint64_t xn%u_ = 0;", q);
            E.line("  nidx_ = pkt_index(kp, g, 0u, ex_begin, ex_count);");
            E.line("  if (nidx_ != NO_PKT) { noff_ = *gp(kp.pkt_off + nidx_); nlen_ = *gp(kp.pkt_len + nidx_); }");
            emit_xpf_issue("  ");
            E.line("  nidx2_ = nidx_ != NO_PKT ? pkt_next(kp, nidx_, 1u, ex_begin, ex_count) : NO_PKT;");
            E.line("  if (nidx2_ != NO_PKT) { noff2_ = *gp(kp.pkt_off + nidx2_); nlen2_ = *gp(kp.pkt_len + nidx2_); }");
        } else if (pf) {
            if (spread_own)
                E.line("  if (!bpre_ && oi_ != NO_PKT) { poff_ = *gp(br_.pkt_off + oi_); plen_ = *gp(br_.pkt_len + oi_); } bpre_ = false;");
            else
                E.line("  uint64_t noff_ = 0; uint32_t nlen_ = 0;");
            if (spread_own) {
            } else if (spread_on)
                E.line("  { const uint32_t n_ = blo_ + threadIdx.x; if (n_ < bhi_) { noff_ = *gp(kp.pkt_off + n_); nlen_ = *gp(kp.pkt_len + n_); } }");
            else
                E.line("  { const uint32_t n_ = pkt_index(kp, g, 0u, ex_begin, ex_count); if (n_ != NO_PKT) { noff_ = *gp(kp.pkt_off + n_); nlen_ = *gp(kp.pkt_len + n_); } }");
        }
        if (spread_own) {
            E.line("  uint32_t oni_ = oi_;   // the thread's next packet");
            E.line("  for (uint32_t j = 0; j < oQ_; j++) {   // the thread's packets of its lane, in order");
            E.line("    const uint32_t i = oni_;");
            E.line("    if (i == NO_PKT) break;");
            E.line("    oni_ = NO_PKT;");
            E.line("    if (j + 1u < oQ_) { const uint64_t x_ = (uint64_t)i + ostr_; if (x_ < olim_) oni_ = (uint32_t)x_; }");
        } else if (spread_on) {
            E.line("  for (uint32_t j = 0; j < SPREAD_PPB / 256u; j++) {");
            E.line("    const uint32_t i = blo_ + j * 256u + threadIdx.x;");
            E.line("    if (i >= bhi_) break;");
        } else {
            E.line("  for (uint32_t j = 0; j < kp.per_lane; j++) {");
            E.line("    uint32_t i;");
            E.line("    if (kp.sched == SCHED_CHUNKED) { const uint64_t ii = (uint64_t)g * kp.per_lane + j; if (ii >= kp.n) break; i = (uint32_t)ii; }");
            E.line("    else if (kp.sched == SCHED_INTERLEAVED) { const uint64_t ii = (uint64_t)j * kp.lanes + (g >= kp.sched_shift ? g - kp.sched_shift : g + kp.lanes - kp.sched_shift); if (ii >= kp.n) break; i = (uint32_t)ii; }");
            E.line("    else { if (j >= ex_count) break; i = ld_nt(kp.sched_pkts + ex_begin + j); }");
        }
        if (lpf_on) {
            E.line("    uint64_t poff_; uint32_t plen_;");
            for (uint32_t q = 0; q < xpf.words; q++) E.line("    uint64_t xc%u_ = 0;", q);
            E.line("    if (j < lpf_n_) {   // parked in LDS when the lane started");
            E.line("      poff_ = lpfo_[j * 256u + threadIdx.x];");
            E.line("      const uint32_t lw_ = lpfl_[j * 256u + threadIdx.x];");
            E.line("      plen_ = lw_ & 0x7fffffffu;");
            E.line("      xc_ok_ = lw_ >> 31;");
            for (uint32_t q = 0; q < xpf.words; q++)
                E.line("      if (xc_ok_) xc%u_ = lpfw_[(j * %uu + %uu) * 256u + threadIdx.x];", q, xpf.words, q);
            E.line("    } else {");
            E.line("      poff_ = *gp(kp.pkt_off + i); plen_ = *gp(kp.pkt_len + i); xc_ok_ = 0u;");
            E.line("    }");
        } else if (pf && xpf.on) {
            E.line("    const uint64_t poff_ = noff_; const uint32_t plen_ = nlen_;");
            E.line("    xc_ok_ = xn_ok_;");
            for (uint32_t q = 0; q < xpf.words; q++) E.line("    const uint64_t xc%u_ = xn%u_;", q, q);
            E.line("    noff_ = noff2_; nlen_ = nlen2_; nidx_ = nidx2_;");
            emit_xpf_issue("    ");
            E.line("    nidx2_ = nidx_ != NO_PKT ? pkt_next(kp, nidx_, j + 2u, ex_begin, ex_count) : NO_PKT;");
            E.line("    if (nidx2_ != NO_PKT) { noff2_ = *gp(kp.pkt_off + nidx2_); nlen2_ = *gp(kp.pkt_len + nidx2_); }");
        } else if (pf) {
            if (!spread_own) E.line("    const uint64_t poff_ = noff_; const uint32_t plen_ = nlen_;");
            if (spread_own) {
                E.line("    if (j + 1u < oQ_) { if (oni_ != NO_PKT) { noff_ = *gp(br_.pkt_off + oni_); nlen_ = *gp(br_.pkt_len + oni_); } }");
                E.line("    else if (bt_ + 1u < nb_ && oi_ != NO_PKT) { const BatchRef &nx_ = obr_[bt_ + 1u]; noff_ = *gp(nx_.pkt_off + oi_); nlen_ = *gp(nx_.pkt_len + oi_); bpre_ = true; }");
            }
            else if (spread_on) E.line("    { const uint32_t n_ = i + 256u; if (n_ < bhi_) { noff_ = *gp(kp.pkt_off + n_); nlen_ = *gp(kp.pkt_len + n_); } }");
            else E.line("    { const uint32_t n_ = pkt_next(kp, i, j + 1, ex_begin, ex_count); if (n_ != NO_PKT) { noff_ = *gp(kp.pkt_off + n_); nlen_ = *gp(kp.pkt_len + n_); } }");
        }
        E.line("    const KParams &kq_ = kp;");
        if (spread_own) {
            E.line("    { const uint32_t ol_ = ochk_ ? i / oP_ : olane_;");
            E.line("      srow_ = ol_ - blockIdx.x * oR_;");
            E.line("      L.cpu = (int32_t)(ocpu_ - olane_ + ol_);");
            E.line("      sbase_ = SM_.backing_addr + (uint32_t)L.cpu * SM_.addr_period; }");
        } else if (spread_on) {
            E.line("    { if (kp.sched == SCHED_CHUNKED) lam_ = i / kp.per_lane;");
            E.line("      else if (j) { lam_ += lstep_; if (lam_ >= kp.cpu_lanes) lam_ -= kp.cpu_lanes; }");
            E.line("      L.cpu = (int32_t)(kp.vcpu_begin + lam_);");
            E.line("      srow_ = lam_ >= lam0_ ? lam_ - lam0_ : lam_ + kp.cpu_lanes - lam0_;");
            E.line("      sbase_ = SM_.backing_addr + (uint32_t)L.cpu * SM_.addr_period; }");
        }
        if (ctx == CTX_SKB) {
            E.line("    uint64_t r1 = 0;");
            if (skb_lds)
                E.line("    const int ls_ = skb_load_lds(kp, L, i, r1, srec_ + %uu * threadIdx.x);", kSrecQ);
            else
                E.line("    const int ls_ = skb_load(kp, L, i, r1);");
        } else {
            if (spread_own) {
                E.line("    uint32_t H = 0u, T = 0u;");
                E.line("    L.ingress = oin_; L.rxq = orx_; L.egress = oeg_;");
                E.line("    if (ofl_) {");
                E.line("      H = kq_.headroom_arr ? ld_nt(kq_.headroom_arr + i) : kq_.headroom;");
                E.line("      T = kq_.tailroom_arr ? ld_nt(kq_.tailroom_arr + i) : kq_.tailroom;");
                E.line("      if (kq_.ingress_arr) L.ingress = (uint32_t)ld_nt(kq_.ingress_arr + i);");
                E.line("      if (kq_.rxq_arr) L.rxq = (uint32_t)ld_nt(kq_.rxq_arr + i);");
                E.line("      if (kq_.egress_arr) L.egress = (uint32_t)ld_nt(kq_.egress_arr + i);");
                E.line("    }");
            } else {
            E.line("    const uint32_t H = kq_.headroom_arr ? ld_nt(kq_.headroom_arr + i) : kq_.headroom;");
            E.line("    const uint32_t T = kq_.tailroom_arr ? ld_nt(kq_.tailroom_arr + i) : kq_.tailroom;");
            }
            if (pf) {
                E.line("    const uint32_t len = plen_;");
                E.line("    L.pkt = %s + poff_;", spread_own ? "br_.pkt_data" : "kq_.pkt_data");
            } else if (spread_own) {
                E.line("    const uint32_t len = *gp(br_.pkt_len + i);");
                E.line("    L.pkt = br_.pkt_data + *gp(br_.pkt_off + i);");
            } else {
                E.line("    const uint32_t len = *gp(kq_.pkt_len + i);");
                E.line("    L.pkt = kq_.pkt_data + *gp(kq_.pkt_off + i);");
            }
            E.line("    L.M = H + len + T;");
            E.line("    L.pa = P;");
            E.line("    L.rec = nullptr;");
            if (spread_own) E.line("    if (ofl_) {");
            E.line("    for (uint32_t b = 0; b < H; b++) *gp(L.pkt + b) = 0;");
            E.line("    for (uint32_t b = 0; b < T; b++) *gp(L.pkt + H + len + b) = 0;");
            if (spread_own) E.line("    }");
            E.line("    L.data = P + H;");
            E.line("    L.data_end = P + H + len;");
            if (!spread_own) {
            E.line("    L.ingress = (uint32_t)(kq_.ingress_arr ? ld_nt(kq_.ingress_arr + i) : kq_.ingress);");
            E.line("    L.rxq = (uint32_t)(kq_.rxq_arr ? ld_nt(kq_.rxq_arr + i) : kq_.rxq);");
            E.line("    L.egress = (uint32_t)(kq_.egress_arr ? ld_nt(kq_.egress_arr + i) : kq_.egress);");
            }
            E.line("    uint64_t r1 = P + L.M + 1;");
        }
        E.line("    SM0(L) = 0; SM1(L) = 0; L.xdp_dirty = 0; L.nframes = 0; L.tailcalls = 0; L.t_lo = 0; L.t_n = 0; L.t_ptr = nullptr;");
        E.line("    uint64_t r0 = 0, r2 = 0, r3 = 0, r4 = 0, r5 = 0, r6 = 0, r7 = 0, r8 = 0, r9 = 0;");
        if (spread_own) E.line("    uint32_t lr10_ = or10_; asm volatile(\"\" : \"+s\"(lr10_));");
        E.line("    uint64_t r10 = %s;", spread_own ? "lr10_" : "kp.static_next + kp.frame_size");
        E.line("    uint32_t steps = 0;");
        if (census) E.line("    coldn_ = 0;");
        if (!spec_use.empty()) E.line("    spv_ = 1;");
        E.line("    int st_ = 0;");
        E.line("    int32_t epc_ = -1;");
        if (proc) E.line("    uint32_t pg_ = kp.entry_prog;");
        if (ctx == CTX_SKB) E.line("    if (ls_) TERM(ls_, -1);");
        if (ctx_check) E.line("    { const uint32_t cz_ = ctx_done(kq_, i); if (cz_) TERM(MIMIC_ERR_CANCELED - 1u + cz_, 0); }");
        if (dispatch_on()) {
            E.line("    uint32_t cur_;   // no initializer: the TERM gotos above jump past it");
            E.line("    cur_ = %s;", spread_own ? "oep_" : "kp.entry_prog");
            E.line("    switch (cur_) {");
            for (auto &p : P)
                if (p.n == 0) E.line("    case %u: steps = 1; TERM(MIMIC_ERR_PC_OOB, 0);", p.id);
            E.line("%s", nonempty_cases().c_str());
            E.line("      break;");
            E.line("    default: TERM(MIMIC_ERR_PC_OOB, 0);");
            E.line("    }");
            E.line("  D_:");
            E.line("    switch (cur_) {");
            for (auto &p : P)
                if (p.n) E.line("    case %u: goto P%u_0;", p.id, p.id);
            E.line("    default: TERM(MIMIC_ERR_ENGINE_HELPER, -1);");
            E.line("    }");
        } else {
            E.line("    switch (%s) {", spread_own ? "oep_" : "kp.entry_prog");
            for (auto &p : P) {
                if (p.n == 0) E.line("    case %u: steps = 1; TERM(MIMIC_ERR_PC_OOB, 0);", p.id);
                else E.line("    case %u: goto P%u_0;", p.id, p.id);
            }
            E.line("    default: TERM(MIMIC_ERR_PC_OOB, 0);");
            E.line("    }");
        }
        for (auto &p : P) program(p);
        E.line("    TERM(MIMIC_ERR_ENGINE_HELPER, -1);");
        if (defer_mode) {
            E.line("  L_defer:");
            E.line("    VC_FLUSH();");
            E.line("    defer_finish(kp, L, g, i, j, lane_steps);");
            E.line("    break;");
        }
        E.line("  L_term:");
        if (spread_own && pf) E.line("    poff_ = noff_; plen_ = nlen_; asm volatile(\"\" : \"+v\"(poff_), \"+v\"(plen_));");
        E.line("    {");
        {
            const char *rb = spread_own ? "lb_" : "kq_";
            if (spread_own) E.line("    const BatchRef &lb_ = obr_[bt_];");
            if (ntres) {
                E.line("    if (%s.r0) st_nt(%s.r0 + i, r0);", rb, rb);
                E.line("    if (%s.status) st_nt(%s.status + i, (uint8_t)st_);", rb, rb);
            } else {
                E.line("    if (%s.r0) *gp(%s.r0 + i) = r0;", rb, rb);
                E.line("    if (%s.status) *gp(%s.status + i) = (uint8_t)st_;", rb, rb);
            }
            if (census) E.line("    if (%s.steps) st_nt(%s.steps + i, coldn_);   // census: slow-path calls, not steps", rb, rb);
            else E.line("    if (%s.steps) st_nt(%s.steps + i, steps);", rb, rb);
            E.line("    if (%s.err_pc) st_nt(%s.err_pc + i, epc_);", rb, rb);
        }
        E.line("    }");
        if (proc) {
            E.line("    if (kq_.step) { StepState *S_ = kq_.step;");
            E.line("      S_->r[0] = r0; S_->r[1] = r1; S_->r[2] = r2; S_->r[3] = r3; S_->r[4] = r4; S_->r[5] = r5;");
            E.line("      S_->r[6] = r6; S_->r[7] = r7; S_->r[8] = r8; S_->r[9] = r9; S_->r[10] = r10;");
            E.line("      S_->pc = epc_; S_->prog = pg_; S_->steps = steps; S_->status = st_; S_->started = 1u; S_->finished = 1u; }");
        }
        E.line("    lane_steps += steps;");
        E.line("  }");
        if (spread_own) E.line("  }   // batches");
        if (vc_on) E.line("  VC_FLUSH();");
        if (spread_own) {
            E.line("  __syncthreads();");
            E.line("  if (ofw_ && sacc_[threadIdx.x]) *ofd_ = ofv_ + sacc_[threadIdx.x];");
            E.line("  for (uint32_t w_ = threadIdx.x + 256u; w_ < oR_ * SPREAD_ROWW; w_ += 256u) {   // rows past 256 words");
            E.line("    const spread_t v_ = sacc_[w_];");
            E.line("    if (!v_) continue;");
            E.line("    const uint32_t r_ = w_ / SPREAD_ROWW, q_ = w_ - r_ * SPREAD_ROWW;");
            E.line("    GAS spread_t *d_ = (GAS spread_t *)(kp.arena + SM_.dev_off + (size_t)(kp.vcpu_begin + blockIdx.x * oR_ + r_) * SM_.dev_stride) + q_;");
            E.line("    *d_ += v_;");
            E.line("  }");
        } else if (spread_on) {
            E.line("#if SPREAD_ROWS");
            E.line("  __syncthreads();");
            E.line("  if (kp.spread_part && kp.cpu_lanes == SPREAD_ROWS) {");
            E.line("    spread_t *pt_ = (spread_t *)kp.spread_part + (size_t)blockIdx.x * (SPREAD_ROWS * SPREAD_ROWW);");
            E.line("    for (uint32_t w_ = threadIdx.x; w_ < SPREAD_ROWS * SPREAD_ROWW; w_ += 256u) {");
            E.line("      const uint32_t r_ = w_ / SPREAD_ROWW, q_ = w_ - r_ * SPREAD_ROWW;");
            E.line("      const uint32_t lr_ = lam0_ + r_ < SPREAD_ROWS ? lam0_ + r_ : lam0_ + r_ - SPREAD_ROWS;");
            E.line("      pt_[lr_ * SPREAD_ROWW + q_] = sacc_[w_];");
            E.line("    }");
            E.line("  } else");
            E.line("  for (uint32_t w_ = threadIdx.x; w_ < SPREAD_ROWS * SPREAD_ROWW; w_ += 256u) {");
            E.line("    const spread_t v_ = sacc_[w_];");
            E.line("    if (!v_) continue;");
            E.line("    const uint32_t r_ = w_ / SPREAD_ROWW, q_ = w_ - r_ * SPREAD_ROWW;");
            E.line("    const uint32_t lr_ = lam0_ + r_ < kp.cpu_lanes ? lam0_ + r_ : lam0_ + r_ - kp.cpu_lanes;");
            E.line("    spread_t *d_ = (spread_t *)(kp.arena + SM_.dev_off + (size_t)(kp.vcpu_begin + lr_) * SM_.dev_stride) + q_;");
            E.line("    __hip_atomic_fetch_add((GAS spread_t *)d_, v_, __ATOMIC_RELAXED, __HIP_MEMORY_SCOPE_AGENT);");
            E.line("  }");
            E.line("#endif");
        }
        E.line("  if (kp.lane_steps) st_nt(kp.lane_steps + g, lane_steps);");
        if (hash_chunk) E.line("  h_chunk_fini();   // the block's last wave hands its chunk's remainder back");
        E.line("}");
        if (spread_own) {
            std::string hs;
            char b[512];
            for (uint32_t s : own_k) {
                snprintf(b, sizeof b, "  uint64_t hk%u_ = cget(kp.insns, %uu).k; asm volatile(\"\" : \"+s\"(hk%u_));\n", s, s, s);
                hs += b;
            }
            for (uint32_t s : own_h) {
                snprintf(b, sizeof b, "  uint32_t hh%u_ = AUX_MAPHINT(cget(kp.insns, %uu).aux); asm volatile(\"\" : \"+s\"(hh%u_));\n", s, s, s);
                hs += b;
            }
            if (!hs.empty()) hs.pop_back();
            const size_t q = E.s.find(kOwnHoist);
            E.s.replace(q, strlen(kOwnHoist), hs);
        }
        if (census) {
            static const char *kinds[] = {"cold_load(", "cold_store(", "cold_lookup(", "cold_update(", "cold_delete(",
                                          "cold_tailcall(", "cold_ldabs(", "cold_adjust_tail("};
            for (int k = 0; k < 8; k++) {
                const std::string from = std::string("COLD_CALL(") + kinds[k], to = "COLD_CALL_K(" + std::to_string(4 * k) + ", " + kinds[k];
                for (size_t q = E.s.find(from); q != std::string::npos; q = E.s.find(from, q + to.size())) E.s.replace(q, from.size(), to);
            }
        }
// ... 1414 lines not shown
```

mimic_amd/csrc/layout.h:

```cpp
#pragma once
#include <stdint.h>
#if defined(__HIPCC__) || defined(__HIP__) || defined(__HIPCC_RTC__)
#define HHD_LAYOUT static __host__ __device__ inline
#else
#define HHD_LAYOUT static inline
#endif

#define MIMIC_MAX_FRAMES 32u
#define MIMIC_DEFAULT_BUDGET (1ull << 22)
#define MIMIC_MEM_START 0x10000u
#define MIMIC_PC_BITS 24u
#define MIMIC_XDP_MD_SIZE 24u
#define MIMIC_FRAME_QWORDS 5u

enum SegKind : uint32_t {
    SEG_PLAIN = 1,
    SEG_ARRAY_OBJ = 2,
    SEG_MAP_OBJ = 3,
    SEG_PROG = 4,
    SEG_PERCPU_ARRAY = 5,
    SEG_PERCPU_VALUES = 6,
};

enum MapFamily : uint32_t { FAM_ARRAY = 1, FAM_PERCPU_ARRAY = 2, FAM_HASH = 3, FAM_PERCPU_HASH = 4 };
// ... 29 lines not shown
};
#define HT_F_CHUNK 1u
#define HT_CHUNK_MAXE (1u << 17)
#define HT_LEFT_CAP 16384u

#define HT_USED_SHARDS 16
struct HashCtl {
    unsigned long long head;
    uint32_t comb_fault;
    uint32_t pad0[29];
    unsigned long long tail;
    int32_t avail;
    uint32_t used0;
    uint32_t pad1[28];
    uint32_t used_sh[HT_USED_SHARDS * 32];
    uint32_t cminv;
    uint32_t full;
    uint32_t cdone;
    uint32_t nleft;
    uint32_t pad2[28];
    uint32_t live_sh[HT_USED_SHARDS * 32];
};
HHD_LAYOUT uint64_t ht_ext_bytes(uint32_t E) {
    const uint64_t e32 = ((uint64_t)E + 1023) & ~1023ull;
    return e32 + e32 * 4 + (uint64_t)HT_LEFT_CAP * 8;
}
#define HT_EMPTY 0xffffffffu
#define HT_TOMB 0xfffffffeu
#define HT_BUSY 0xfffffffdu

struct DProg {
    uint32_t base;
    uint32_t n;
    uint32_t addr;
    uint32_t pad;
};

enum Handler : uint32_t {
    H_SLOW = 0,
    H_ERR = 1,
    H_NOP = 2,
    H_ALU64 = 3,
    H_ALU32 = 4,
    H_LDIMM = 5,
    H_JA = 6,
    H_JCC = 7,
    H_LDX = 8,
    H_ST = 9,
    H_STX = 10,
    H_EXIT = 11,
    H_CALL = 12,
    H_CALL_LOCAL = 13,
    H_LDABS = 14,
};
#define AUX_H(a) ((a) & 0xffu)
#define AUX_FALL_OK (1u << 8)
#define AUX_JT_OK (1u << 9)
#define AUX_JT_NEG (1u << 10)
#define AUX_W32 (1u << 11)
#define AUX_X (1u << 12)
#define AUX_ARG(a) (((a) >> 16) & 0xffu)
#define AUX_SZ(a) ((a) >> 24)
#define AUX_MAPHINT(a) ((a) >> 16)
struct DInsn {
    uint32_t w;
    uint32_t aux;
    uint64_t k;
};

enum Sched : uint32_t { SCHED_CHUNKED = 0, SCHED_INTERLEAVED = 1, SCHED_EXPLICIT = 2 };

enum CtxKind : uint32_t { CTX_XDP = 0, CTX_SKB = 1 };
struct SkbRec;

#define MIMIC_MANY_MAX 8u
struct BatchRef {
    uint8_t *pkt_data;
    const uint64_t *pkt_off;
    const uint32_t *pkt_len;
    uint64_t *r0;
    uint8_t *status;
    uint32_t *steps;
    int32_t *err_pc;
    uint64_t pad;
};

struct KParams {
    const DInsn *insns;
    const DProg *progs;
    const Seg *segs;
    const DMap *maps;
    uint8_t *arena;
    uint32_t nprogs, nsegs, nmaps, entry_prog;
    uint32_t static_next;
    uint32_t stack_size;
    uint32_t frame_size;
    uint32_t chunk_shift;
    uint32_t max_tail_calls;
    uint32_t total_vcpus;
    uint32_t vcpu_begin;
    uint32_t lanes;
    uint32_t priv_lanes;
    uint8_t *priv;
    uint32_t priv_xdp_q;
    uint32_t priv_frame_q;
    uint32_t priv_key_q;
    uint32_t cpu_lanes;
    uint64_t budget;
    uint32_t n;
    uint32_t sched;
    uint32_t per_lane;
    uint32_t sched_shift;
    uint8_t *pkt_data;
    const uint64_t *pkt_off;
    const uint32_t *pkt_len;
    const uint32_t *headroom_arr;
    const uint32_t *tailroom_arr;
    const int32_t *ingress_arr;
    const int32_t *rxq_arr;
    const int32_t *egress_arr;
    uint32_t headroom, tailroom;
    int32_t ingress, rxq, egress;
    uint32_t step_gen;
    const uint32_t *sched_start;
    const uint32_t *sched_pkts;
    uint64_t *r0;
    uint8_t *status;
    uint32_t *steps;
    int32_t *err_pc;
    uint64_t *lane_steps;
    uint32_t ctx_kind;
    uint32_t skb_ifindex;
    SkbRec *skb_rec;
    const uint64_t *skb_prefix;
    const uint64_t *skb_base;
    struct StepState *step;
    uint32_t hash_pop_only;
    uint32_t hash_ro;
    struct DeferRec *defer;
    uint32_t *defer_any;
    uint32_t defer_epoch;
    uint32_t reserved0;
    uint32_t *spread_bad;
    const void *skb_custom;
    const uint64_t *skb_drv;
    void *spread_part;
    const uint32_t *cancel;
    const uint32_t *const *cancel_pp;
    uint32_t cancel_any;
    uint32_t own_q;
    uint32_t many_n;
    struct BatchRef many[MIMIC_MANY_MAX];
    const uint8_t *step_img;
    uint8_t *step_dst;
    uint32_t step_img_n;
    uint32_t step_ins_n;
    uint32_t *skb_rooms_state;
};
static_assert(sizeof(KParams) == 968, "KParams: the kernarg layout of every JIT kernel");
static_assert(__builtin_offsetof(KParams, reserved0) == 356 && __builtin_offsetof(KParams, spread_bad) == 360,
              "KParams: the fields around the reserved word keep their offsets");

struct DeferRec {
    uint64_t r[11];
    int32_t pc;
    uint32_t prog;
    uint32_t steps;
    uint32_t j;
    uint64_t lane_steps;
    uint64_t sm0, sm1;
    uint32_t xdp_dirty, nframes, tailcalls;
    uint32_t flag;
};

struct StepState {
    uint64_t r[11];
    int32_t pc;
    uint32_t prog;
    uint32_t steps;
    int32_t status;
    uint32_t started;
    uint32_t finished;
    int32_t cpu;
    uint32_t gen;
    uint8_t lane[256];
};
```

mimic_amd/csrc/runtime.h:

```cpp
#pragma once
#include <stdint.h>

#include "layout.h"
#include "hashmap.h"
#include "skb.h"
#include "../../include/mimic_amd.h"

typedef uint16_t __attribute__((aligned(1))) u16u;
typedef uint32_t __attribute__((aligned(1))) u32u;
typedef uint64_t __attribute__((aligned(1))) u64u;

#define DEV static __device__ __forceinline__
#ifndef MIMIC_HASH_NOLOCK
#define MIMIC_HASH_NOLOCK 1
#endif
#ifdef MIMIC_HASH_POPONLY
#define HASH_POPONLY(kp) (MIMIC_HASH_POPONLY != 0)
#else
#define HASH_POPONLY(kp) ((kp).hash_pop_only != 0)
#endif
#ifdef MIMIC_HASH_RO
#define HASH_RO(kp) (MIMIC_HASH_RO != 0)
#else
#define HASH_RO(kp) ((kp).hash_ro != 0)
#endif

#define CONST_AS __attribute__((address_space(4)))
template <typename T>
DEV T cget(const T *p, uint32_t i) {
    static_assert(sizeof(T) % 4 == 0, "dword-sized tables only");
    uint32_t w[sizeof(T) / 4];
#if defined(__HIP_DEVICE_COMPILE__)
    const CONST_AS uint32_t *q = (const CONST_AS uint32_t *)(p + i);
#else
    const uint32_t *q = (const uint32_t *)(p + i);
#endif
#pragma unroll
    for (unsigned k = 0; k < sizeof(T) / 4; k++) w[k] = q[k];
    T out;
    __builtin_memcpy(&out, w, sizeof(T));
    return out;
}

enum RegionKind : uint32_t {
    RK_UNRES = 0, RK_STACK = 1, RK_XDP = 2, RK_GLOBAL = 3, RK_NOTVMMEM = 4, RK_NOTDATASEC = 5,
    RK_SKB = 6, RK_SK = 7, RK_FK = 8,
    RK_BEPKT = 9
};

#ifdef MIMIC_CTX_FIXED
#define CTX_SKB_MODE(kp) (MIMIC_CTX_FIXED == CTX_SKB)
#else
#define CTX_SKB_MODE(kp) ((kp).ctx_kind == CTX_SKB)
#endif

struct Ref {
    uint32_t rk, off, limit;
    int32_t map, sub, prog;
    uint8_t *ptr;
};

struct Lane {
    uint32_t lane;
    int32_t cpu;
    uint32_t M;
    uint8_t *pkt;
    uint32_t data, data_end, ingress, rxq, egress;
    uint32_t xdp_dirty;
    uint64_t sm0, sm1;
    uint32_t nframes, tailcalls;
    uint32_t t_lo, t_n;
    uint8_t *t_ptr;
    uint32_t pa;
    uint32_t ka;
    SkbRec *rec;
};

static constexpr int EXIT_SIG = -1;

DEV int32_t lane_cpu(const KParams &kp, uint32_t g) {
    if (g < kp.cpu_lanes) return (int32_t)(kp.vcpu_begin + g);
    return g == kp.cpu_lanes ? -1 : (int32_t)kp.total_vcpus;
}

#if defined(__HIP_DEVICE_COMPILE__)
#define GAS __attribute__((address_space(1)))
#else
#define GAS
#endif
template <typename T>
DEV GAS T *gp(T *p) { return (GAS T *)p; }

DEV uint32_t ctx_done(const KParams &kp, uint32_t i) {
    const uint32_t *w = kp.cancel_pp ? kp.cancel_pp[i] : kp.cancel;
    if (!w) return 0u;
    return __hip_atomic_load((GAS const uint32_t *)w, __ATOMIC_RELAXED, __HIP_MEMORY_SCOPE_SYSTEM);
}
template <typename T>
DEV const GAS T *gp(const T *p) { return (const GAS T *)p; }

#define NO_PKT 0xffffffffu
DEV uint32_t pkt_index(const KParams &kp, uint32_t g, uint32_t j, uint32_t ex_begin, uint32_t ex_count) {
    if (j >= kp.per_lane) return NO_PKT;
    if (kp.sched == SCHED_CHUNKED) {
        const uint64_t ii = (uint64_t)g * kp.per_lane + j;
        return ii < kp.n ? (uint32_t)ii : NO_PKT;
    }
    if (kp.sched == SCHED_INTERLEAVED) {
        const uint64_t ii = (uint64_t)j * kp.lanes + (g >= kp.sched_shift ? g - kp.sched_shift : g + kp.lanes - kp.sched_shift);
        return ii < kp.n ? (uint32_t)ii : NO_PKT;
    }
    return j < ex_count ? *(const GAS uint32_t *)(kp.sched_pkts + ex_begin + j) : NO_PKT;
}

DEV uint32_t spread_lane(const KParams &kp, uint32_t i) {
    if (kp.sched == SCHED_CHUNKED) return i / kp.per_lane;
    uint32_t r = i % kp.cpu_lanes + kp.sched_shift;
    return r >= kp.cpu_lanes ? r - kp.cpu_lanes : r;
}

DEV uint32_t pkt_next(const KParams &kp, uint32_t i, uint32_t j, uint32_t ex_begin, uint32_t ex_count) {
    if (j >= kp.per_lane) return NO_PKT;
    if (kp.sched == SCHED_EXPLICIT) return j < ex_count ? *(const GAS uint32_t *)(kp.sched_pkts + ex_begin + j) : NO_PKT;
    const uint64_t ii = (uint64_t)i + (kp.sched == SCHED_CHUNKED ? 1u : kp.lanes);
    return ii < kp.n ? (uint32_t)ii : NO_PKT;
}

DEV uint64_t ld_n(const uint8_t *p, uint32_t n) {
    switch (n) {
    case 1: return *gp(p);
    case 2: return *(const GAS u16u *)p;
    case 4: return *(const GAS u32u *)p;
    case 8: return *(const GAS u64u *)p;
    default: {
        uint64_t v = 0;
        for (uint32_t i = n; i-- > 0;) v = (v << 8) | *gp(p + i);
        return v;
    }
    }
}
DEV void st_n(uint8_t *p, uint32_t n, uint64_t v) {
    switch (n) {
    case 1: *gp(p) = (uint8_t)v; return;
    case 2: *(GAS u16u *)p = (uint16_t)v; return;
    case 4: *(GAS u32u *)p = (uint32_t)v; return;
    case 8: *(GAS u64u *)p = v; return;
    default:
        for (uint32_t i = 0; i < n; i++) *gp(p + i) = (uint8_t)(v >> (8 * i));
    }
}

template <typename T>
DEV T ld_nt(const T *p) { return __builtin_nontemporal_load(gp(p)); }
template <typename T>
DEV void st_nt(T *p, T v) { __builtin_nontemporal_store(v, gp(p)); }

DEV uint64_t vc_sel(uint32_t q, uint64_t w0, uint64_t w1, uint64_t w2, uint64_t w3) {
    return q == 0 ? w0 : q == 1 ? w1 : q == 2 ? w2 : q == 3 ? w3 : 0ull;
}
DEV uint64_t vc_load(uint64_t w0, uint64_t w1, uint64_t w2, uint64_t w3, uint32_t o, uint32_t n) {
    const uint32_t q = o >> 3, sh = (o & 7) * 8;
    const uint64_t lo = vc_sel(q, w0, w1, w2, w3);
    uint64_t v = lo;
    if (sh) v = (lo >> sh) | (vc_sel(q + 1, w0, w1, w2, w3) << (64 - sh));
    return n >= 8 ? v : (v & ((1ull << (8 * n)) - 1));
}
DEV void vc_store(uint64_t &w0, uint64_t &w1, uint64_t &w2, uint64_t &w3, uint32_t o, uint32_t n, uint64_t v) {
    const uint32_t q = o >> 3, sh = (o & 7) * 8;
    const uint64_t m = n >= 8 ? ~0ull : ((1ull << (8 * n)) - 1);
    v &= m;
    const uint64_t lm = m << sh, lv = v << sh;
    const uint64_t hm = sh ? m >> (64 - sh) : 0ull, hv = sh ? v >> (64 - sh) : 0ull;
    w0 = q == 0 ? ((w0 & ~lm) | lv) : w0;
    w1 = q == 1 ? ((w1 & ~lm) | lv) : q == 0 ? ((w1 & ~hm) | hv) : w1;
    w2 = q == 2 ? ((w2 & ~lm) | lv) : q == 1 ? ((w2 & ~hm) | hv) : w2;
    w3 = q == 3 ? ((w3 & ~lm) | lv) : q == 2 ? ((w3 & ~hm) | hv) : w3;
}

DEV uint8_t *priv_b(const KParams &kp, uint32_t lane, uint32_t o) {
    return kp.priv + (((size_t)(o >> 3) * kp.priv_lanes + lane) << 3) + (o & 7);
}
DEV uint64_t priv_load(const KParams &kp, uint32_t lane, uint32_t o, uint32_t n) {
// ... 612 lines not shown
    const HT t = h_table(kp.arena, m);
    h_delete_wave(t, ks, h);
    o.r0 = 0;
    o.set_r0 = true;
    return o;
}

DEV HelperOut helper_tailcall(const KParams &kp, const Lane &L, uint64_t r2, uint64_t r3) {
    HelperOut o = {0, 0, false, false, 0, 0, 0, nullptr};
    if (L.tailcalls >= kp.max_tail_calls) {
        o.r0 = (uint64_t)(int64_t)-1;
        o.set_r0 = true;
        return o;
    }
    int32_t mid, sub;
    if (!reg_to_map(kp, L, r2, mid, sub)) { o.st = MIMIC_ERR_HELPER_MAP_PTR; return o; }
    const DMap m = load_map(kp, mid);
    if (m.type != MIMIC_MAP_PROG_ARRAY || m.key_size != 4 || m.family != FAM_ARRAY) {
        o.st = MIMIC_ERR_HELPER_TAILCALL;
        return o;
    }
    uint32_t slot = array_value_addr(m, -1, (uint32_t)r3);
    Ref R = resolve(kp, L, slot);
    if (R.rk == RK_UNRES) {
        o.r0 = (uint64_t)(int64_t)-22;
        o.set_r0 = true;
        return o;
    }
    if (!is_vmmem(R.rk)) { o.st = MIMIC_ERR_HELPER_TAILCALL; return o; }
    uint64_t pa = 0;
    if (mem_load(kp, L, R, 4, pa)) pa = 0;
    Ref P = resolve(kp, L, (uint32_t)pa);
    if (P.prog < 0) {
        o.r0 = (uint64_t)(int64_t)-22;
        o.set_r0 = true;
        return o;
    }
    o.tail = true;
    o.new_prog = (uint32_t)P.prog;
    return o;
}

DEV int helper_class(int32_t n) {
    switch (n) {
    case 4: case 14: case 15: case 16: case 17: case 22: case 24: case 27: case 35: case 36: case 42:
    case 45: case 46: case 47: case 55: case 56: case 67: case 69: case 80: case 112: case 113: case 114:
    case 115: case 119: case 120: case 122: case 123: case 128: case 129: case 141: case 148: case 151:
        return 2;
    case 1: case 2: case 3: case 5: case 7: case 8: case 9: case 12: case 25: case 38: case 65: case 87:
    case 88: case 89: case 125: case 160:
        return 1;
    default:
        return 0;
    }
}

DEV int ld_abs(const KParams &kp, const Lane &L, uint64_t r6, uint32_t x, uint32_t n, bool bad_src, uint64_t &v) {
    const Ref S = resolve(kp, L, (uint32_t)r6);
    if (S.rk != RK_SKB) return MIMIC_ERR_LDABS;
    if (bad_src) return MIMIC_PANIC_BADREG;
    const Ref P = resolve(kp, L, L.pa + SKB_HEADROOM + x);
    if (!is_vmmem(P.rk)) return MIMIC_ERR_LDABS;
    const int rc = mem_load(kp, L, P, n, v);
    if (rc == MIMIC_PANIC_SLICE) return rc;
    return rc ? MIMIC_ERR_LDABS : 0;
}

DEV void skb_rooms_zero(uint8_t *pkt, uint32_t lw) {
    typedef uint64_t u64x2u __attribute__((ext_vector_type(2), aligned(1)));
    const u64x2u z = {0, 0};
    GAS u64x2u *hw = (GAS u64x2u *)pkt, *tw = (GAS u64x2u *)(pkt + SKB_HEADROOM + lw);
    hw[0] = z;
    hw[1] = z;
    for (uint32_t q = 0; q < SKB_TAILROOM / 16; q++) tw[q] = z;
}
DEV bool skb_rec_dirty(const SkbRec &r) { return r.ip[0].pad[0] != 0; }
static_assert(SKB_HEADROOM == 32 && SKB_TAILROOM == 64, "skb_rooms_zero covers 2 + 4 16-byte chunks");

DEV uint64_t skb_leak_pre(const KParams &kp, uint32_t i) {
    return (kp.skb_prefix[i] & SKB_PFX_MASK) + kp.skb_prefix[kp.n + (i >> SKB_PREP_LOG2)];
}
DEV int skb_load(const KParams &kp, Lane &L, uint32_t i, uint64_t &r1, bool attach_only = false) {
    SkbRec *rec = kp.skb_rec + i;
    L.pkt = kp.pkt_data + kp.pkt_off[i];
    const uint64_t pf = kp.skb_prefix[i];
    if (kp.skb_drv && !attach_only)
        for (uint32_t q = 0; q < SKB_DERIVED_Q; q++) ((uint64_t *)rec)[q] = kp.skb_drv[(size_t)i * SKB_DERIVED_Q + q];
    const uint32_t lw = rec->len;
    L.rec = nullptr;
    L.ka = 0;
    L.pa = 0;
    L.M = 0;
    if (lw & SKB_LOAD_FAILED) return MIMIC_ERR_CTX_LOAD;
    const uint64_t ka = *kp.skb_base + skb_leak_pre(kp, i);
    if (ka + SKB_FOOT_FIXED - 1 + lw > 0xffffffffull) return MIMIC_ERR_CTX_LOAD;
    if (!attach_only) {
        for (uint32_t q = 0; q < 8; q++) ((uint64_t *)rec)[SKB_DERIVED_Q + q] = skb_writable_word(q);
        skb_apply_custom(*rec, (const mimic_skb_custom *)kp.skb_custom, i);
    }
    L.rec = rec;
    L.ka = (uint32_t)ka;
    L.pa = L.ka + SKB_SK_SIZE + 1 + SKB_FK_SIZE + 1;
    L.M = SKB_HEADROOM + lw + SKB_TAILROOM;
    if (!attach_only && (pf & SKB_PFX_DIRTY)) skb_rooms_zero(L.pkt, lw);
    r1 = kp.static_next + kp.stack_size + 1;
    return 0;
}

DEV int skb_attach(const KParams &kp, Lane &L, uint32_t i, uint64_t &r1, uint64_t *d, uint32_t lw, uint64_t pre, uint64_t base,
                   int dirty) {
    skb_apply_custom(*(SkbRec *)d, (const mimic_skb_custom *)kp.skb_custom, i);
    L.rec = nullptr;
    L.ka = 0;
    L.pa = 0;
    L.M = 0;
    if (lw & SKB_LOAD_FAILED) return MIMIC_ERR_CTX_LOAD;
    const uint64_t ka = base + pre;
    if (ka + SKB_FOOT_FIXED - 1 + lw > 0xffffffffull) return MIMIC_ERR_CTX_LOAD;
    L.rec = (SkbRec *)d;
    L.ka = (uint32_t)ka;
    L.pa = L.ka + SKB_SK_SIZE + 1 + SKB_FK_SIZE + 1;
    L.M = SKB_HEADROOM + lw + SKB_TAILROOM;
    if (dirty) skb_rooms_zero(L.pkt, lw);
    r1 = kp.static_next + kp.stack_size + 1;
    return 0;
}

DEV int skb_load_lds(const KParams &kp, Lane &L, uint32_t i, uint64_t &r1, uint64_t *d) {
    const uint64_t po = kp.pkt_off[i];
    typedef uint64_t u64x2a __attribute__((ext_vector_type(2)));
    const GAS u64x2a *s = (const GAS u64x2a *)(kp.skb_drv + (size_t)i * SKB_DERIVED_Q);
    uint64_t w[SKB_DERIVED_Q];
#pragma unroll
    for (uint32_t q = 0; q < SKB_DERIVED_Q / 2; q++) {
        const u64x2a v = s[q];
        w[2 * q] = v.x;
        w[2 * q + 1] = v.y;
    }
    const uint64_t pre = skb_leak_pre(kp, i), base = *kp.skb_base;
#pragma unroll
    for (uint32_t q = 0; q < SKB_DERIVED_Q; q++) d[q] = w[q];
#pragma unroll
    for (uint32_t q = 0; q < 8; q++) d[SKB_DERIVED_Q + q] = skb_writable_word(q);
    L.pkt = kp.pkt_data + po;
    return skb_attach(kp, L, i, r1, d, (uint32_t)w[0], pre, base, (int)((w[SKB_DIRTY_Q] >> SKB_DIRTY_SHIFT) & 1u));
}

struct Spill {
    Lane L;
    uint64_t r[11];
    uint64_t v;
    int32_t st;
    uint32_t po;
    uint32_t tail;
    uint32_t new_prog;
};
DEV void atomic_add_n(uint8_t *p, uint32_t n, uint64_t v) {
    if (n == 8) __hip_atomic_fetch_add((GAS uint64_t *)p, v, __ATOMIC_RELAXED, __HIP_MEMORY_SCOPE_WORKGROUP);
    else __hip_atomic_fetch_add((GAS uint32_t *)p, (uint32_t)v, __ATOMIC_RELAXED, __HIP_MEMORY_SCOPE_WORKGROUP);
}

DEV void defer_finish(const KParams &kp, const Lane &L, uint32_t g, uint32_t i, uint32_t j, uint64_t lane_steps) {
    DeferRec *d = kp.defer + g;
    if (L.rec && L.rec != kp.skb_rec + i) {
        const uint64_t *s = (const uint64_t *)L.rec;
        GAS uint64_t *o = (GAS uint64_t *)(kp.skb_rec + i);
        for (uint32_t q = 0; q < sizeof(SkbRec) / 8; q++) o[q] = s[q];
    }
#ifdef MIMIC_LDS_STACK_Q
    for (uint32_t q = 0; q < MIMIC_LDS_STACK_Q; q++) {
        const uint32_t o = STK_LDS_LO + 8u * q;
        if (stk_valid(kp, L, o)) *gp((uint64_t *)priv_b(kp, L.lane, o)) = stk_lw(o);
    }
#endif
    d->sm0 = SM0(L);
    d->sm1 = SM1(L);
    d->xdp_dirty = L.xdp_dirty;
    d->nframes = L.nframes;
    d->tailcalls = L.tailcalls;
    d->j = j;
    d->lane_steps = lane_steps;
    d->flag = kp.defer_epoch;
    *gp(kp.defer_any) = kp.defer_epoch;
}

#if defined(MIMIC_COLD_INLINE) && MIMIC_COLD_INLINE
#define COLD DEV
#define COLD_OPAQUE() do { } while (0)
#else
#define COLD static __device__ __attribute__((noinline, cold))
#define COLD_OPAQUE() asm volatile("" ::: "memory")
#endif
COLD void cold_load(const KParams &kp, Spill &S, uint32_t a, uint32_t n) {
    COLD_OPAQUE();
    S.v = 0;
    S.st = mem_load(kp, S.L, resolve(kp, S.L, a), n, S.v);
}
COLD void cold_store(const KParams &kp, Spill &S, uint32_t a, uint32_t n, uint64_t v) {
    COLD_OPAQUE();
    const Ref R = resolve(kp, S.L, a);
    S.st = mem_store(kp, S.L, R, n, v);
    S.po = (!S.st && R.ptr == S.L.pkt && (R.rk == RK_GLOBAL || R.rk == RK_BEPKT)) ? R.off + 1 : 0;
}
DEV void cold_take(Spill &S, const HelperOut &ho) {
    S.st = ho.st;
    if (!ho.st && ho.set_r0) S.r[0] = ho.r0;
}
COLD void cold_lookup(const KParams &kp, Spill &S) {
    COLD_OPAQUE();
    const HelperOut ho = helper_lookup(kp, S.L, S.r[1], S.r[2]);
    cold_take(S, ho);
    if (!ho.st && ho.t_n) {
// ... 234 lines not shown
```

mimic_amd/vm.py:

```python
from __future__ import annotations

import base64
import ctypes as C
import json
import os
from dataclasses import dataclass, field
from enum import IntEnum
from typing import Dict, Iterable, List, Optional, Sequence, Tuple

from . import _lib as L


class MimicError(RuntimeError):
    pass


class MapType(IntEnum):
    Hash = 1
    Array = 2
    ProgramArray = 3
    PerfEventArray = 4
    PerCPUHash = 5
    PerCPUArray = 6

# ... 754 lines not shown
        pkt = bytes(ctx.Packet)
        if isinstance(ctx, LinuxContextSKBuff):
            cust = skb_custom_record(ctx)
            cp = cust.ctypes.data if int(cust["flags"]) else None
            _check(self.VM.h, self.VM.lib.mimic_process_new_skb_ctx(self.VM.h, self.prog_id, pkt, len(pkt),
                                                                     ctx.Dev.IFIndex if ctx.Dev else 0, cp, C.byref(h)),
                   "NewProcess")
        else:
            _check(self.VM.h, self.VM.lib.mimic_process_new(self.VM.h, self.prog_id, pkt, len(pkt), ctx.Headroom,
                                                             ctx.Tailroom, ctx.IngessIfIndex, ctx.RxQueueIndex,
                                                             ctx.EgressIfIndex, C.byref(h)), "NewProcess")
        self._native = h
        if self.cpuID >= 0:
            _check(self.VM.h, self.VM.lib.mimic_process_set_cpu(h, self.cpuID), "SetCPUID")

    def _take(self, regs) -> None:
        for q in range(11):
            setattr(self.Registers, f"R{q}", int(regs.r[q]))
        self.Registers.PC = int(regs.pc)
        self.ProgramID = int(regs.prog_id)
        self.Steps = int(regs.steps)
        self.Status = int(regs.status)
        self._exited = bool(regs.exited)

    def Step(self) -> bool:
        self._ensure_native()
        self._started = True
        regs = L.ProcessRegs()
        rc = self.VM.lib.mimic_process_step(self._native, 1, C.byref(regs))
        if rc < 0:
            _check(self.VM.h, rc, "Step")
        self._take(regs)
        if self.Status:
            self.ErrPC = self.Registers.PC
            raise MimicError(f"inst at PC({self.Registers.PC}): {L.STATUS_NAMES[self.Status]}")
        return self._exited

    def Run(self, step_budget: int = 0, ctx: Optional["Context"] = None) -> None:
        self._ensure_native()
        self._started = True
        regs = L.ProcessRegs()
        if ctx is not None:
            rc = self.VM.lib.mimic_process_run_ctx(self._native, step_budget, ctx._device_handle(), C.byref(regs))
            if rc in (L.ECANCELED, L.EDEADLINE):
                self._take(regs)
                raise MimicError(Context._ERR[1 if rc == L.ECANCELED else 2])
            _check(self.VM.h, rc, "Run")
        else:
            _check(self.VM.h, self.VM.lib.mimic_process_run(self._native, step_budget, C.byref(regs)), "Run")
        self._take(regs)
        self.ErrPC = self.Registers.PC if self.Status else -1
        self.PacketAfter = self.Packet()
        if self.Status:
            raise MimicError(f"process encountered a fatal error: {L.STATUS_NAMES[self.Status]} at PC({self.ErrPC})")

    def Packet(self) -> bytes:
        if self._native is None:
            return self.PacketAfter or b""
        ctx = self.Context or LinuxContextXDP()
        if isinstance(ctx, LinuxContextSKBuff):
            n = 32 + len(ctx.Packet) + 64
        else:
            n = ctx.Headroom + len(ctx.Packet) + ctx.Tailroom
        buf = C.create_string_buffer(max(n, 1))
        _check(self.VM.h, self.VM.lib.mimic_process_packet(self._native, buf, max(n, 1)), "packet")
        return buf.raw[:n]

    def Cleanup(self) -> None:
        if self._native is not None and getattr(self.VM, "h", None):
            self.VM.lib.mimic_process_free(self._native)
        self._native = None

    def __del__(self):
        try:
            self.Cleanup()
        except Exception:
            pass



class XDPBatch:

    def __init__(self, pkt_data, pkt_off, pkt_len, headroom=0, tailroom=0, ingress=0, rxq=0, egress=0,
                 schedule=L.SCHED_CHUNKED, cpu=None, step_budget=0):
        self.pkt_data, self.pkt_off, self.pkt_len = pkt_data, pkt_off, pkt_len
        self.headroom, self.tailroom = headroom, tailroom
        self.ingress, self.rxq, self.egress = ingress, rxq, egress
        self.schedule, self.cpu, self.step_budget = schedule, cpu, step_budget

    @property
    def n(self) -> int:
        return int(self.pkt_len.numel())

    def _c(self):
        cached = getattr(self, "_cstruct", None)
        if cached is not None:
            return cached
        import torch

        b = L.XDPBatch()
        b.n = self.n
        b.schedule = self.schedule
        b.pkt_data = self.pkt_data.data_ptr()
        b.pkt_off = self.pkt_off.data_ptr()
        b.pkt_len = self.pkt_len.data_ptr()
        b.headroom = self.headroom.data_ptr() if isinstance(self.headroom, torch.Tensor) else None
        b.headroom_all = 0 if isinstance(self.headroom, torch.Tensor) else int(self.headroom)
        b.tailroom = self.tailroom.data_ptr() if isinstance(self.tailroom, torch.Tensor) else None
        b.tailroom_all = 0 if isinstance(self.tailroom, torch.Tensor) else int(self.tailroom)
        for fld, allname, val in (("ingress_ifindex", "ingress_all", self.ingress), ("rx_queue_index", "rxq_all", self.rxq),
                                  ("egress_ifindex", "egress_all", self.egress)):
            if isinstance(val, torch.Tensor):
                setattr(b, fld, val.data_ptr())
                setattr(b, allname, 0)
            else:
                setattr(b, fld, None)
                setattr(b, allname, int(val))
        self._cpu_host = None
        if self.schedule == L.SCHED_EXPLICIT:
            import numpy as np

            self._cpu_host = np.ascontiguousarray(np.asarray(self.cpu, dtype=np.int32))
            b.cpu = self._cpu_host.ctypes.data
        else:
            b.cpu = None
        b.step_budget = self.step_budget
        self._cstruct = C.byref(b)
        self._cstruct_obj = b
        return self._cstruct

    @staticmethod
    def layout(lengths: Sequence[int], headroom=0, tailroom=0, align: int = 64):
        import numpy as np

        lens = np.asarray(lengths, dtype=np.int64)
        H = np.asarray(headroom, dtype=np.int64) if not np.isscalar(headroom) else np.full(lens.shape, headroom)
        T = np.asarray(tailroom, dtype=np.int64) if not np.isscalar(tailroom) else np.full(lens.shape, tailroom)
        sizes = (H + lens + T + align - 1) // align * align
        off = np.zeros(lens.shape, dtype=np.int64)
        if len(lens) > 1:
            off[1:] = np.cumsum(sizes)[:-1]
        total = int(sizes.sum()) if len(lens) else 0
        return off.astype(np.uint64), total

    @classmethod
    def from_packets(cls, packets: Sequence[bytes], device="cuda", headroom=0, tailroom=0, ingress=0, rxq=0,
                     egress=0, schedule=L.SCHED_CHUNKED, cpu=None, step_budget=0):
        import numpy as np
        import torch

        lens = [len(p) for p in packets]
        H_arr = None if np.isscalar(headroom) else np.asarray(headroom, dtype=np.uint32)
        T_arr = None if np.isscalar(tailroom) else np.asarray(tailroom, dtype=np.uint32)
        off, total = cls.layout(lens, headroom, tailroom)
        buf = np.zeros(max(total, 1), dtype=np.uint8)
        for i, p in enumerate(packets):
            h = int(H_arr[i]) if H_arr is not None else int(headroom)
            buf[int(off[i]) + h:int(off[i]) + h + len(p)] = np.frombuffer(bytes(p), dtype=np.uint8)
        return cls.from_numpy(buf, off, np.asarray(lens, dtype=np.uint32), device, H_arr if H_arr is not None
                              else headroom, T_arr if T_arr is not None else tailroom, ingress, rxq, egress,
                              schedule, cpu, step_budget)

    @classmethod
    def from_numpy(cls, buf, off, lens, device="cuda", headroom=0, tailroom=0, ingress=0, rxq=0, egress=0,
                   schedule=L.SCHED_CHUNKED, cpu=None, step_budget=0):
        import numpy as np
        import torch

        def t(a, dt):
            return torch.from_numpy(np.ascontiguousarray(np.asarray(a, dtype=dt))).to(device)

        def opt(v, dt):
            return v if np.isscalar(v) else t(v, dt)

        return cls(t(buf, np.uint8), t(np.asarray(off, dtype=np.uint64).view(np.int64), np.int64),
                   t(np.asarray(lens, dtype=np.uint32).view(np.int32), np.int32),
                   opt(headroom, np.int32), opt(tailroom, np.int32), opt(ingress, np.int32), opt(rxq, np.int32),
                   opt(egress, np.int32), schedule, cpu, step_budget)

    def packet_bytes(self, i: int) -> bytes:
        import numpy as np

        o = int(self.pkt_off[i].item())
        h = int(self.headroom[i].item()) if not np.isscalar(self.headroom) else int(self.headroom)
        t_ = int(self.tailroom[i].item()) if not np.isscalar(self.tailroom) else int(self.tailroom)
        n = h + int(self.pkt_len[i].item()) + t_
        return bytes(self.pkt_data[o:o + n].cpu().numpy().tobytes())


class SKBBatch:
    HEADROOM, TAILROOM = 32, 64

    def __init__(self, pkt_data, pkt_off, pkt_len, ifindex=0, schedule=L.SCHED_CHUNKED, cpu=None, step_budget=0,
                 custom=None):
        self.pkt_data, self.pkt_off, self.pkt_len = pkt_data, pkt_off, pkt_len
        self.ifindex, self.schedule, self.cpu, self.step_budget = ifindex, schedule, cpu, step_budget
        self.custom = custom

    @property
    def n(self) -> int:
        return int(self.pkt_len.numel())

    def _c(self):
        cached = getattr(self, "_cstruct", None)
        if cached is not None:
            return cached
        b = L.SKBBatch()
        b.n, b.schedule = self.n, self.schedule
        b.pkt_data, b.pkt_off, b.pkt_len = self.pkt_data.data_ptr(), self.pkt_off.data_ptr(), self.pkt_len.data_ptr()
        b.ifindex = int(self.ifindex)
        self._cpu_host = None
        if self.schedule == L.SCHED_EXPLICIT:
            import numpy as np

            self._cpu_host = np.ascontiguousarray(np.asarray(self.cpu, dtype=np.int32))
            b.cpu = self._cpu_host.ctypes.data
        else:
            b.cpu = None
        b.step_budget = self.step_budget
        b.custom = self.custom.data_ptr() if self.custom is not None else None
        if getattr(self, "rooms_state", None) is None:
            import torch

            self.rooms_state = torch.zeros(1, dtype=torch.int32, device=self.pkt_data.device)
        b.rooms_state = self.rooms_state.data_ptr()
        self._cstruct_obj = b
        self._cstruct = C.byref(b)
        return self._cstruct

    def PacketsWritten(self) -> None:
        if getattr(self, "rooms_state", None) is not None:
            self.rooms_state.zero_()

    @classmethod
    def layout(cls, lengths: Sequence[int], align: int = 64):
        return XDPBatch.layout(lengths, cls.HEADROOM, cls.TAILROOM, align)

    @staticmethod
    def custom_array(contexts: Sequence["LinuxContextSKBuff"]):
        import numpy as np

        recs = np.zeros(len(contexts), L.SKB_CUSTOM_DTYPE)
        for i, c in enumerate(contexts):
            recs[i] = skb_custom_record(c)
        return recs if recs["flags"].any() else None

    @classmethod
    def from_packets(cls, packets: Sequence[bytes], device="cuda", ifindex=0, schedule=L.SCHED_CHUNKED, cpu=None,
                     step_budget=0, custom=None):
        import numpy as np

        lens = np.asarray([len(p) for p in packets], dtype=np.uint32)
        off, total = cls.layout(lens)
        buf = np.zeros(max(total, 1), dtype=np.uint8)
        for i, p in enumerate(packets):
            o = int(off[i]) + cls.HEADROOM
            buf[o:o + len(p)] = np.frombuffer(bytes(p), dtype=np.uint8)
        return cls.from_numpy(buf, off, lens, device, ifindex, schedule, cpu, step_budget, custom)

    @classmethod
    def from_numpy(cls, buf, off, lens, device="cuda", ifindex=0, schedule=L.SCHED_CHUNKED, cpu=None, step_budget=0,
                   custom=None):
        import numpy as np
        import torch

        def t(a, dt):
            return torch.from_numpy(np.ascontiguousarray(np.asarray(a, dtype=dt))).to(device)

        cu = None
# ... 241 lines not shown
    def _run(self, jobs) -> None:
        V = self.vm.settings.vcpus
        groups: Dict[Tuple[int, bool, int], list] = {}
        owner: Dict[int, Tuple[int, bool, int]] = {}
        for job in jobs:
            err = job.Context.Err() if job.Context is not None else None
            if err is not None:
                self._handoff(job, MimicError(err))
                continue
            cpu = self._next_cpu
            skb = isinstance(job.Process.Context, LinuxContextSKBuff)
            ifx = (job.Process.Context.Dev.IFIndex if job.Process.Context.Dev else 0) if skb else 0
            key = (job.Process.prog_id, skb, ifx)
            if owner.get(cpu, key) != key:
                self._run_groups(groups)
                groups, owner = {}, {}
            if skb and not job.Process._started:
                job.Process.cpuID = cpu
            else:
                job.Process.SetCPUID(cpu)
            self._next_cpu = (cpu + 1) % V
            owner[cpu] = key
            groups.setdefault(key, []).append(job)
        self._run_groups(groups)

    def _run_groups(self, groups) -> None:
        for (pid, skb, _ifx), js in groups.items():
            try:
                self._launch(pid, skb, js)
            except MimicError as ex:
                for job in js:
                    self._handoff(job, ex)
                continue
            done = []
            for job in js:
                p = job.Process
                err = None
                if p.Status in (L.STATUS["ERR_CANCELED"], L.STATUS["ERR_DEADLINE"]):
                    err = MimicError(Context._ERR[p.Status - L.STATUS["ERR_CANCELED"] + 1])
                elif p.Status:
                    err = MimicError(f"process encountered a fatal error: {L.STATUS_NAMES[p.Status]} at PC({p.ErrPC})")
                if job.Handoff is None:
                    done.append(p)
                else:
                    self._handoff(job, err)
            self.vm.CleanupProcesses(done)

    def _launch(self, pid: int, skb: bool, js) -> None:
        dev = f"cuda:{self.vm.settings.device}"
        ctxs = [j.Process.Context or LinuxContextXDP() for j in js]
        cpus = [j.Process.cpuID for j in js]
        if skb:
            fresh = []
            for j in js + [None]:
                if j is not None and not j.Process._started:
                    fresh.append(j)
                    continue
                if fresh:
                    self.vm.RunProcesses([f.Process for f in fresh], [f.Context for f in fresh],
                                         [f.Process.cpuID for f in fresh])
                    fresh = []
                if j is None:
                    break
                try:
                    j.Process.Run(ctx=j.Context)
                except MimicError as ex:
                    if str(ex) in Context._ERR.values():
                        j.Process.Status = L.STATUS["ERR_CANCELED"] + (str(ex) == Context._ERR[2])
                    elif not j.Process.Status:
                        raise
            return
        import numpy as np

        hr = [c.Headroom for c in ctxs]
        batch = XDPBatch.from_packets([c.Packet for c in ctxs], device=dev, headroom=np.array(hr, np.uint32),
                                      tailroom=np.array([c.Tailroom for c in ctxs], np.uint32),
                                      ingress=np.array([c.IngessIfIndex for c in ctxs], np.int32),
                                      rxq=np.array([c.RxQueueIndex for c in ctxs], np.int32),
                                      egress=np.array([c.EgressIfIndex for c in ctxs], np.int32),
                                      schedule=L.SCHED_EXPLICIT, cpu=cpus)
        cpp = [j.Context for j in js] if any(j.Context is not None for j in js) else None
        res = self.vm.RunXDPBatch(pid, batch, ctx_per_packet=cpp).numpy(len(js))
        mem = batch.pkt_data.cpu().numpy()
        offs = batch.pkt_off.cpu().numpy()
        for k, j in enumerate(js):
            p = j.Process
            p.Registers.R0 = int(res["r0"][k]) & 0xFFFFFFFFFFFFFFFF
            p.Steps = int(res["steps"][k])
            p.Status = int(res["status"][k])
            p.ErrPC = int(res["err_pc"][k])
            c = ctxs[k]
            tail = c.Tailroom
            o = int(offs[k])
            p.PacketAfter = bytes(mem[o:o + hr[k] + len(c.Packet) + tail].tobytes())
```

Measured before the change: 62470 Mpkts/s.

## Drop per-packet offset/length arrays for uniformly strided, equal-length XDP batches

Adds pkt_stride and pkt_len_all fields to the XDP batch descriptor. When offsets form an arithmetic sequence and all lengths are equal, the Python builder omits the pkt_off and pkt_len arrays. The JIT kernels then compute offset = i*stride and use a constant length instead of loading per-packet descriptors. This removes descriptor memory traffic and prefetch loads from the packet loop. The cost is extra flag checks and branches in the generated code, plus an ABI struct-size change.

```diff
diff --git a/include/mimic_amd.h b/include/mimic_amd.h
--- a/include/mimic_amd.h
+++ b/include/mimic_amd.h
@@ -110,6 +110,8 @@
     const int32_t *egress_ifindex;  int32_t egress_all;
     const int32_t *cpu;
     uint64_t step_budget;
+    uint32_t pkt_stride;
+    uint32_t pkt_len_all;
 } mimic_xdp_batch;
 
 typedef struct {
@@ -120,6 +122,7 @@
 } mimic_xdp_results;
 
 int mimic_abi_version(void);
+int mimic_xdp_batch_size(void);
 const char *mimic_last_error(const mimic_vm *vm);
 
 int mimic_vm_create(const mimic_vm_settings *settings, mimic_vm **out);
diff --git a/mimic_amd/_lib.py b/mimic_amd/_lib.py
--- a/mimic_amd/_lib.py
+++ b/mimic_amd/_lib.py
@@ -52,7 +52,8 @@
                 ("ingress_ifindex", C.c_void_p), ("ingress_all", C.c_int32),
                 ("rx_queue_index", C.c_void_p), ("rxq_all", C.c_int32),
                 ("egress_ifindex", C.c_void_p), ("egress_all", C.c_int32),
-                ("cpu", C.c_void_p), ("step_budget", C.c_uint64)]
+                ("cpu", C.c_void_p), ("step_budget", C.c_uint64),
+                ("pkt_stride", C.c_uint32), ("pkt_len_all", C.c_uint32)]
 
 
 class SKBBatch(C.Structure):
@@ -95,6 +96,7 @@
 
 EXPORTS = {
     "mimic_abi_version": (C.c_int, []),
+    "mimic_xdp_batch_size": (C.c_int, []),
     "mimic_last_error": (C.c_char_p, [C.c_void_p]),
     "mimic_vm_create": (C.c_int, [C.POINTER(VMSettings), C.POINTER(C.c_void_p)]),
     "mimic_vm_destroy": (None, [C.c_void_p]),
@@ -192,5 +194,7 @@
         fn.argtypes = args
     if lib.mimic_abi_version() != ABI_VERSION:
         raise ImportError("libmimic_amd.so ABI version mismatch")
+    if lib.mimic_xdp_batch_size() != C.sizeof(XDPBatch):
+        raise ImportError("libmimic_amd.so: sizeof(mimic_xdp_batch) differs from the binding's")
     _lib = lib
     return lib
diff --git a/mimic_amd/csrc/engine.cpp b/mimic_amd/csrc/engine.cpp
--- a/mimic_amd/csrc/engine.cpp
+++ b/mimic_amd/csrc/engine.cpp
@@ -606,6 +606,7 @@
 extern "C" {
 
 int mimic_abi_version(void) { return MIMIC_ABI_VERSION; }
+int mimic_xdp_batch_size(void) { return (int)sizeof(mimic_xdp_batch); }
 
 const char *mimic_last_error(const mimic_vm *vm) { return vm ? vm->err.c_str() : "null vm"; }
 
@@ -1547,6 +1548,15 @@
                         hipStream_t st_in, uint64_t shift, const SkbRun *skb = nullptr, const StepRun *step = nullptr,
                         const CtxRun *cx = nullptr, ManyRun *mr = nullptr);
 
+static int xdp_batch_check(mimic_vm *vm, const mimic_xdp_batch *b, int64_t at) {
+    const char *why = nullptr;
+    if (b->n > 0 && !b->pkt_data) why = "missing packet memory";
+    else if (b->n > 1 && !b->pkt_off && !b->pkt_stride) why = "no pkt_off and pkt_stride 0: every packet at the same address";
+    if (!why) return 0;
+    if (at < 0) return fail(vm, MIMIC_EINVAL, "%s", why);
+    return fail(vm, MIMIC_EINVAL, "batch %lld: %s", (long long)at, why);
+}
+
 int mimic_run_xdp(mimic_vm *vm, uint32_t prog_id, const mimic_xdp_batch *b, const mimic_xdp_results *res,
                   void *hip_stream) {
     return run_xdp_impl(vm, prog_id, b, res, (hipStream_t)hip_stream, 0);
@@ -1556,6 +1566,9 @@
                        void *hip_stream) {
     if (!vm || (k && (!b || !res))) return MIMIC_EINVAL;
     hipStream_t st = (hipStream_t)hip_stream;
+    if (k && prog_id >= vm->progs.size()) return fail(vm, MIMIC_EINVAL, "no program with id '%u' is loaded", prog_id);
+    for (uint32_t q = 0; q < k; q++)
+        if (const int rc = xdp_batch_check(vm, b + q, q)) return rc;
     auto same = [&](const mimic_xdp_batch &x, const mimic_xdp_batch &y) {
         return x.n == y.n && x.schedule == y.schedule && x.schedule != MIMIC_SCHED_EXPLICIT && !x.headroom && !y.headroom &&
                !x.tailroom && !y.tailroom && !x.ingress_ifindex && !y.ingress_ifindex && !x.rx_queue_index &&
@@ -1827,7 +1840,8 @@
                         const CtxRun *cx, ManyRun *mr) {
     if (!vm || !b || !res) return MIMIC_EINVAL;
     if (prog_id >= vm->progs.size()) return fail(vm, MIMIC_EINVAL, "no program with id '%u' is loaded", prog_id);
-    if (b->n > 0 && (!b->pkt_data || !b->pkt_off || !b->pkt_len)) return fail(vm, MIMIC_EINVAL, "missing packet arrays");
+    if (const int brc = xdp_batch_check(vm, b, -1)) return brc;
+    if (skb && b->n > 0 && (!b->pkt_off || !b->pkt_len)) return fail(vm, MIMIC_EINVAL, "missing packet arrays");
     if (cx && cx->all && cx->per_packet) return fail(vm, MIMIC_EINVAL, "one context for the batch or one per packet, not both");
     if (cx && cx->all && !cx->all->pinned) return fail(vm, MIMIC_EDEVICE, "the context was made without a device");
     if (cx && cx->per_packet)
@@ -1909,6 +1923,8 @@
     kp.pkt_data = b->pkt_data;
     kp.pkt_off = b->pkt_off;
     kp.pkt_len = b->pkt_len;
+    kp.pkt_stride = b->pkt_off ? 0u : b->pkt_stride;
+    kp.pkt_len_all = b->pkt_len ? 0u : b->pkt_len_all;
     kp.headroom_arr = b->headroom;
     kp.tailroom_arr = b->tailroom;
     kp.ingress_arr = b->ingress_ifindex;
@@ -2191,9 +2207,12 @@
         mr->used = jit && own && !ji.defer && mr->k >= 1 && mr->k <= MIMIC_MANY_MAX;
         if (mr->used) {
             kp.many_n = mr->k;
-            for (uint32_t q = 0; q < mr->k; q++)
-                kp.many[q] = BatchRef{mr->b[q].pkt_data, mr->b[q].pkt_off, mr->b[q].pkt_len, mr->r[q].r0, mr->r[q].status,
-                                      mr->r[q].steps, mr->r[q].err_pc, 0};
+            for (uint32_t q = 0; q < mr->k; q++) {
+                const mimic_xdp_batch &bq = mr->b[q];
+                kp.many[q] = BatchRef{bq.pkt_data, bq.pkt_off, bq.pkt_len, mr->r[q].r0, mr->r[q].status, mr->r[q].steps,
+                                      mr->r[q].err_pc,
+                                      (bq.pkt_off ? 0u : bq.pkt_stride) | (uint64_t)(bq.pkt_len ? 0u : bq.pkt_len_all) << 32};
+            }
         }
     }
     if (jit) {
diff --git a/mimic_amd/csrc/interp.hip b/mimic_amd/csrc/interp.hip
--- a/mimic_amd/csrc/interp.hip
+++ b/mimic_amd/csrc/interp.hip
@@ -32,7 +32,10 @@
         const uint64_t lines = (spans[k][1] + 63) / 64;
         for (uint64_t q = t; q < lines && q < 4096; q += nt) n += *(const volatile uint32_t *)(spans[k][0] + q * 64);
     }
-    if (t == 0) n += *(const volatile uint32_t *)kp.pkt_off + *(const volatile uint32_t *)kp.pkt_len;
+    if (t == 0) {
+        if (kp.pkt_off) n += *(const volatile uint32_t *)kp.pkt_off;
+        if (kp.pkt_len) n += *(const volatile uint32_t *)kp.pkt_len;
+    }
     (void)n;
 }
 #define NREGS 11
@@ -173,8 +176,8 @@
         } else if (i != 0xffffffffu) {
             const uint32_t H = kp.headroom_arr ? kp.headroom_arr[i] : kp.headroom;
             const uint32_t T = kp.tailroom_arr ? kp.tailroom_arr[i] : kp.tailroom;
-            const uint32_t len = kp.pkt_len[i];
-            L.pkt = kp.pkt_data + kp.pkt_off[i];
+            const uint32_t len = pkt_len_at(kp, i);
+            L.pkt = kp.pkt_data + pkt_off_at(kp, i);
             L.M = H + len + T;
             if (!resume_here) {
                 for (uint32_t b = 0; b < H; b++) L.pkt[b] = 0;
diff --git a/mimic_amd/csrc/jit.cpp b/mimic_amd/csrc/jit.cpp
--- a/mimic_amd/csrc/jit.cpp
+++ b/mimic_amd/csrc/jit.cpp
@@ -319,7 +319,7 @@
             E.line("  __shared__ spread_t sacc_[SPREAD_ROWS * SPREAD_ROWW];");
             E.line("  for (uint32_t w_ = threadIdx.x; w_ < SPREAD_ROWS * SPREAD_ROWW; w_ += 256u) sacc_[w_] = 0;");
             E.line("  __shared__ BatchRef obr_[MIMIC_MANY_MAX];");
-            E.line("  if (threadIdx.x < (kp.many_n ? kp.many_n : 1u)) obr_[threadIdx.x] = kp.many_n ? cget(kp.many, threadIdx.x) : BatchRef{kp.pkt_data, kp.pkt_off, kp.pkt_len, kp.r0, kp.status, kp.steps, kp.err_pc, 0};");
+            E.line("  if (threadIdx.x < (kp.many_n ? kp.many_n : 1u)) obr_[threadIdx.x] = kp.many_n ? cget(kp.many, threadIdx.x) : BatchRef{kp.pkt_data, kp.pkt_off, kp.pkt_len, kp.r0, kp.status, kp.steps, kp.err_pc, kp.pkt_stride | (uint64_t)kp.pkt_len_all << 32};");
             E.line("  __syncthreads();");
             E.line("  uint32_t srow_ = orow_, sbase_ = 0;");
             E.line("  const bool ofw_ = threadIdx.x < oR_ * SPREAD_ROWW && blockIdx.x * oR_ + threadIdx.x / SPREAD_ROWW < kp.cpu_lanes;");
@@ -376,7 +376,10 @@
             E.line("  const uint32_t nb_ = kp.many_n ? kp.many_n : 1u;");
             E.line("  bool bpre_ = false;   // this batch's first descriptor came with the previous batch's last packet");
             E.line("  for (uint32_t bt_ = 0; bt_ < nb_; bt_++) {");
-            E.line("  const BatchRef br_ = kp.many_n ? cget(kp.many, bt_) : BatchRef{kp.pkt_data, kp.pkt_off, kp.pkt_len, kp.r0, kp.status, kp.steps, kp.err_pc, 0};");
+            E.line("  const BatchRef br_ = kp.many_n ? cget(kp.many, bt_) : BatchRef{kp.pkt_data, kp.pkt_off, kp.pkt_len, kp.r0, kp.status, kp.steps, kp.err_pc, kp.pkt_stride | (uint64_t)kp.pkt_len_all << 32};");
+            E.line("  uint32_t cstr_ = (uint32_t)br_.compact, clen_ = (uint32_t)(br_.compact >> 32);");
+            E.line("  asm volatile(\"\" : \"+v\"(cstr_), \"+v\"(clen_));");
+            E.line("  ofl_ = (ofl_ & 3u) | (br_.pkt_off ? 0u : 4u) | (br_.pkt_len ? 0u : 8u);");
         }
         if (lpf_on) {
             const uint32_t D = kLpfD, XW = xpf.words;
@@ -390,7 +393,7 @@
             for (uint32_t d = 0; d < D; d++) {
                 E.line("    const uint32_t lx%u_ = pkt_index(kp, g, %uu, ex_begin, ex_count);", d, d);
                 E.line("    uint64_t lo%u_ = 0; uint32_t ll%u_ = 0;", d, d);
-                E.line("    if (lx%u_ != NO_PKT) { lo%u_ = *gp(kp.pkt_off + lx%u_); ll%u_ = *gp(kp.pkt_len + lx%u_); }", d, d, d, d, d);
+                E.line("    if (lx%u_ != NO_PKT) { lo%u_ = pkt_off_at(kp, lx%u_); ll%u_ = pkt_len_at(kp, lx%u_); }", d, d, d, d, d);
             }
             for (uint32_t d = 0; d < D; d++) {
                 for (uint32_t q = 0; q < XW; q++) E.line("    uint64_t lw%u_%u_ = 0;", d, q);
@@ -414,20 +417,26 @@
             E.line("  uint64_t noff_ = 0, noff2_ = 0; uint32_t nlen_ = 0, nlen2_ = 0, nidx_ = NO_PKT, nidx2_ = NO_PKT, xn_ok_ = 0u, xc_ok_ = 0u;");
             for (uint32_t q = 0; q < xpf.words; q++) E.line("  uint64_t xn%u_ = 0;", q);
             E.line("  nidx_ = pkt_index(kp, g, 0u, ex_begin, ex_count);");
-            E.line("  if (nidx_ != NO_PKT) { noff_ = *gp(kp.pkt_off + nidx_); nlen_ = *gp(kp.pkt_len + nidx_); }");
+            E.line("  if (nidx_ != NO_PKT) { noff_ = pkt_off_at(kp, nidx_); nlen_ = pkt_len_at(kp, nidx_); }");
             emit_xpf_issue("  ");
             E.line("  nidx2_ = nidx_ != NO_PKT ? pkt_next(kp, nidx_, 1u, ex_begin, ex_count) : NO_PKT;");
-            E.line("  if (nidx2_ != NO_PKT) { noff2_ = *gp(kp.pkt_off + nidx2_); nlen2_ = *gp(kp.pkt_len + nidx2_); }");
+            E.line("  if (nidx2_ != NO_PKT) { noff2_ = pkt_off_at(kp, nidx2_); nlen2_ = pkt_len_at(kp, nidx2_); }");
         } else if (pf) {
             if (spread_own)
-                E.line("  if (!bpre_ && oi_ != NO_PKT) { poff_ = *gp(br_.pkt_off + oi_); plen_ = *gp(br_.pkt_len + oi_); } bpre_ = false;");
+            {
+                E.line("  if (oi_ != NO_PKT) {");
+                E.line("    if (!bpre_) { pkt_off_pf(!(ofl_ & 4u), br_.pkt_off, oi_, noff_); pkt_len_pf(!(ofl_ & 8u), br_.pkt_len, oi_, nlen_); }");
+                E.line("    poff_ = pkt_off_take(!(ofl_ & 4u), noff_, cstr_, oi_); plen_ = pkt_len_take(!(ofl_ & 8u), nlen_, clen_);");
+                E.line("  }");
+                E.line("  bpre_ = false;");
+            }
             else
                 E.line("  uint64_t noff_ = 0; uint32_t nlen_ = 0;");
             if (spread_own) {
             } else if (spread_on)
-                E.line("  { const uint32_t n_ = blo_ + threadIdx.x; if (n_ < bhi_) { noff_ = *gp(kp.pkt_off + n_); nlen_ = *gp(kp.pkt_len + n_); } }");
+                E.line("  { const uint32_t n_ = blo_ + threadIdx.x; if (n_ < bhi_) pkt_desc_pf(kp, n_, noff_, nlen_); }");
             else
-                E.line("  { const uint32_t n_ = pkt_index(kp, g, 0u, ex_begin, ex_count); if (n_ != NO_PKT) { noff_ = *gp(kp.pkt_off + n_); nlen_ = *gp(kp.pkt_len + n_); } }");
+                E.line("  { const uint32_t n_ = pkt_index(kp, g, 0u, ex_begin, ex_count); if (n_ != NO_PKT) pkt_desc_pf(kp, n_, noff_, nlen_); }");
         }
         if (spread_own) {
             E.line("  uint32_t oni_ = oi_;   // the thread's next packet");
@@ -458,7 +467,7 @@
             for (uint32_t q = 0; q < xpf.words; q++)
                 E.line("      if (xc_ok_) xc%u_ = lpfw_[(j * %uu + %uu) * 256u + threadIdx.x];", q, xpf.words, q);
             E.line("    } else {");
-            E.line("      poff_ = *gp(kp.pkt_off + i); plen_ = *gp(kp.pkt_len + i); xc_ok_ = 0u;");
+            E.line("      poff_ = pkt_off_at(kp, i); plen_ = pkt_len_at(kp, i); xc_ok_ = 0u;");
             E.line("    }");
         } else if (pf && xpf.on) {
             E.line("    const uint64_t poff_ = noff_; const uint32_t plen_ = nlen_;");
@@ -467,15 +476,20 @@
             E.line("    noff_ = noff2_; nlen_ = nlen2_; nidx_ = nidx2_;");
             emit_xpf_issue("    ");
             E.line("    nidx2_ = nidx_ != NO_PKT ? pkt_next(kp, nidx_, j + 2u, ex_begin, ex_count) : NO_PKT;");
-            E.line("    if (nidx2_ != NO_PKT) { noff2_ = *gp(kp.pkt_off + nidx2_); nlen2_ = *gp(kp.pkt_len + nidx2_); }");
+            E.line("    if (nidx2_ != NO_PKT) { noff2_ = pkt_off_at(kp, nidx2_); nlen2_ = pkt_len_at(kp, nidx2_); }");
         } else if (pf) {
-            if (!spread_own) E.line("    const uint64_t poff_ = noff_; const uint32_t plen_ = nlen_;");
+            if (!spread_own) E.line("    const uint64_t poff_ = pkt_off_take(kp, noff_, i); const uint32_t plen_ = pkt_len_take(kp, nlen_);");
             if (spread_own) {
-                E.line("    if (j + 1u < oQ_) { if (oni_ != NO_PKT) { noff_ = *gp(br_.pkt_off + oni_); nlen_ = *gp(br_.pkt_len + oni_); } }");
-                E.line("    else if (bt_ + 1u < nb_ && oi_ != NO_PKT) { const BatchRef &nx_ = obr_[bt_ + 1u]; noff_ = *gp(nx_.pkt_off + oi_); nlen_ = *gp(nx_.pkt_len + oi_); bpre_ = true; }");
-            }
-            else if (spread_on) E.line("    { const uint32_t n_ = i + 256u; if (n_ < bhi_) { noff_ = *gp(kp.pkt_off + n_); nlen_ = *gp(kp.pkt_len + n_); } }");
-            else E.line("    { const uint32_t n_ = pkt_next(kp, i, j + 1, ex_begin, ex_count); if (n_ != NO_PKT) { noff_ = *gp(kp.pkt_off + n_); nlen_ = *gp(kp.pkt_len + n_); } }");
+                E.line("    uint32_t cf_ = ofl_; asm volatile(\"\" : \"+s\"(cf_));");
+                E.line("    const uint64_t *po_ = nullptr; const uint32_t *pl_ = nullptr;");
+                E.line("    if (j + 1u < oQ_) { if (oni_ != NO_PKT && (cf_ & 12u) != 12u) { po_ = (cf_ & 4u) ? (const uint64_t *)&kp : br_.pkt_off + oni_; pl_ = (cf_ & 8u) ? (const uint32_t *)&kp : br_.pkt_len + oni_; } }");
+                E.line("    else if (bt_ + 1u < nb_ && oi_ != NO_PKT) { const BatchRef &nx_ = obr_[bt_ + 1u];");
+                E.line("      if (nx_.pkt_off || nx_.pkt_len) { po_ = nx_.pkt_off ? nx_.pkt_off + oi_ : (const uint64_t *)&kp; pl_ = nx_.pkt_len ? nx_.pkt_len + oi_ : (const uint32_t *)&kp; }");
+                E.line("      bpre_ = true; }");
+                E.line("    if (po_) { pkt_off_pf(true, po_, 0u, noff_); pkt_len_pf(true, pl_, 0u, nlen_); }");
+            }
+            else if (spread_on) E.line("    { const uint32_t n_ = i + 256u; if (n_ < bhi_) pkt_desc_pf(kp, n_, noff_, nlen_); }");
+            else E.line("    { const uint32_t n_ = pkt_next(kp, i, j + 1, ex_begin, ex_count); if (n_ != NO_PKT) pkt_desc_pf(kp, n_, noff_, nlen_); }");
         }
         E.line("    const KParams &kq_ = kp;");
         if (spread_own) {
@@ -500,7 +514,7 @@
             if (spread_own) {
                 E.line("    uint32_t H = 0u, T = 0u;");
                 E.line("    L.ingress = oin_; L.rxq = orx_; L.egress = oeg_;");
-                E.line("    if (ofl_) {");
+                E.line("    if (ofl_ & 3u) {");
                 E.line("      H = kq_.headroom_arr ? ld_nt(kq_.headroom_arr + i) : kq_.headroom;");
                 E.line("      T = kq_.tailroom_arr ? ld_nt(kq_.tailroom_arr + i) : kq_.tailroom;");
                 E.line("      if (kq_.ingress_arr) L.ingress = (uint32_t)ld_nt(kq_.ingress_arr + i);");
@@ -515,16 +529,16 @@
                 E.line("    const uint32_t len = plen_;");
                 E.line("    L.pkt = %s + poff_;", spread_own ? "br_.pkt_data" : "kq_.pkt_data");
             } else if (spread_own) {
-                E.line("    const uint32_t len = *gp(br_.pkt_len + i);");
-                E.line("    L.pkt = br_.pkt_data + *gp(br_.pkt_off + i);");
+                E.line("    const uint32_t len = pkt_len_at(!(ofl_ & 8u), br_.pkt_len, clen_, i);");
+                E.line("    L.pkt = br_.pkt_data + pkt_off_at(!(ofl_ & 4u), br_.pkt_off, cstr_, i);");
             } else {
-                E.line("    const uint32_t len = *gp(kq_.pkt_len + i);");
-                E.line("    L.pkt = kq_.pkt_data + *gp(kq_.pkt_off + i);");
+                E.line("    const uint32_t len = pkt_len_at(kq_, i);");
+                E.line("    L.pkt = kq_.pkt_data + pkt_off_at(kq_, i);");
             }
             E.line("    L.M = H + len + T;");
             E.line("    L.pa = P;");
             E.line("    L.rec = nullptr;");
-            if (spread_own) E.line("    if (ofl_) {");
+            if (spread_own) E.line("    if (ofl_ & 3u) {");
             E.line("    for (uint32_t b = 0; b < H; b++) *gp(L.pkt + b) = 0;");
             E.line("    for (uint32_t b = 0; b < T; b++) *gp(L.pkt + H + len + b) = 0;");
             if (spread_own) E.line("    }");
@@ -583,7 +597,7 @@
             E.line("    break;");
         }
         E.line("  L_term:");
-        if (spread_own && pf) E.line("    poff_ = noff_; plen_ = nlen_; asm volatile(\"\" : \"+v\"(poff_), \"+v\"(plen_));");
+        if (spread_own && pf) E.line("    { uint32_t ct_ = ofl_; asm volatile(\"\" : \"+s\"(ct_)); poff_ = pkt_off_take(!(ct_ & 4u), noff_, cstr_, oni_); plen_ = pkt_len_take(!(ct_ & 8u), nlen_, clen_); asm volatile(\"\" : \"+v\"(poff_), \"+v\"(plen_)); }");
         E.line("    {");
         {
             const char *rb = spread_own ? "lb_" : "kq_";
diff --git a/mimic_amd/csrc/layout.h b/mimic_amd/csrc/layout.h
--- a/mimic_amd/csrc/layout.h
+++ b/mimic_amd/csrc/layout.h
@@ -135,7 +135,7 @@
     uint8_t *status;
     uint32_t *steps;
     int32_t *err_pc;
-    uint64_t pad;
+    uint64_t compact;
 };
 
 struct KParams {
@@ -193,7 +193,7 @@
     struct DeferRec *defer;
     uint32_t *defer_any;
     uint32_t defer_epoch;
-    uint32_t reserved0;
+    uint32_t pkt_stride;
     uint32_t *spread_bad;
     const void *skb_custom;
     const uint64_t *skb_drv;
@@ -203,6 +203,7 @@
     uint32_t cancel_any;
     uint32_t own_q;
     uint32_t many_n;
+    uint32_t pkt_len_all;
     struct BatchRef many[MIMIC_MANY_MAX];
     const uint8_t *step_img;
     uint8_t *step_dst;
@@ -211,8 +212,10 @@
     uint32_t *skb_rooms_state;
 };
 static_assert(sizeof(KParams) == 968, "KParams: the kernarg layout of every JIT kernel");
-static_assert(__builtin_offsetof(KParams, reserved0) == 356 && __builtin_offsetof(KParams, spread_bad) == 360,
-              "KParams: the fields around the reserved word keep their offsets");
+static_assert(__builtin_offsetof(KParams, pkt_stride) == 356 && __builtin_offsetof(KParams, spread_bad) == 360,
+              "KParams: the fields around the once reserved word keep their offsets");
+static_assert(__builtin_offsetof(KParams, pkt_len_all) + 4 == __builtin_offsetof(KParams, many),
+              "KParams: pkt_len_all fills the padding ahead of many[]");
 
 struct DeferRec {
     uint64_t r[11];
diff --git a/mimic_amd/csrc/runtime.h b/mimic_amd/csrc/runtime.h
--- a/mimic_amd/csrc/runtime.h
+++ b/mimic_amd/csrc/runtime.h
@@ -98,6 +98,21 @@
 }
 template <typename T>
 DEV const GAS T *gp(const T *p) { return (const GAS T *)p; }
+
+DEV uint64_t pkt_off_at(bool arr, const uint64_t *off, uint32_t stride, uint32_t i) { return arr ? *gp(off + i) : (uint64_t)i * stride; }
+DEV uint32_t pkt_len_at(bool arr, const uint32_t *len, uint32_t len_all, uint32_t i) { return arr ? *gp(len + i) : len_all; }
+DEV void pkt_off_pf(bool arr, const uint64_t *off, uint32_t i, uint64_t &pf) { if (arr) pf = *gp(off + i); }
+DEV void pkt_len_pf(bool arr, const uint32_t *len, uint32_t i, uint32_t &pf) { if (arr) pf = *gp(len + i); }
+DEV uint64_t pkt_off_take(bool arr, uint64_t pf, uint32_t stride, uint32_t i) { return arr ? pf : (uint64_t)i * stride; }
+DEV uint32_t pkt_len_take(bool arr, uint32_t pf, uint32_t len_all) { return arr ? pf : len_all; }
+DEV void pkt_desc_pf(const KParams &kp, uint32_t i, uint64_t &off_pf, uint32_t &len_pf) {
+    pkt_off_pf(kp.pkt_off != nullptr, kp.pkt_off, i, off_pf);
+    pkt_len_pf(kp.pkt_len != nullptr, kp.pkt_len, i, len_pf);
+}
+DEV uint64_t pkt_off_take(const KParams &kp, uint64_t pf, uint32_t i) { return pkt_off_take(kp.pkt_off != nullptr, pf, kp.pkt_stride, i); }
+DEV uint32_t pkt_len_take(const KParams &kp, uint32_t pf) { return pkt_len_take(kp.pkt_len != nullptr, pf, kp.pkt_len_all); }
+DEV uint64_t pkt_off_at(const KParams &kp, uint32_t i) { return pkt_off_at(kp.pkt_off != nullptr, kp.pkt_off, kp.pkt_stride, i); }
+DEV uint32_t pkt_len_at(const KParams &kp, uint32_t i) { return pkt_len_at(kp.pkt_len != nullptr, kp.pkt_len, kp.pkt_len_all, i); }
 
 #define NO_PKT 0xffffffffu
 DEV uint32_t pkt_index(const KParams &kp, uint32_t g, uint32_t j, uint32_t ex_begin, uint32_t ex_count) {
@@ -876,7 +891,7 @@
 }
 DEV int skb_load(const KParams &kp, Lane &L, uint32_t i, uint64_t &r1, bool attach_only = false) {
     SkbRec *rec = kp.skb_rec + i;
-    L.pkt = kp.pkt_data + kp.pkt_off[i];
+    L.pkt = kp.pkt_data + pkt_off_at(kp, i);
     const uint64_t pf = kp.skb_prefix[i];
     if (kp.skb_drv && !attach_only)
         for (uint32_t q = 0; q < SKB_DERIVED_Q; q++) ((uint64_t *)rec)[q] = kp.skb_drv[(size_t)i * SKB_DERIVED_Q + q];
@@ -921,7 +936,7 @@
 }
 
 DEV int skb_load_lds(const KParams &kp, Lane &L, uint32_t i, uint64_t &r1, uint64_t *d) {
-    const uint64_t po = kp.pkt_off[i];
+    const uint64_t po = pkt_off_at(kp, i);
     typedef uint64_t u64x2a __attribute__((ext_vector_type(2)));
     const GAS u64x2a *s = (const GAS u64x2a *)(kp.skb_drv + (size_t)i * SKB_DERIVED_Q);
     uint64_t w[SKB_DERIVED_Q];
diff --git a/mimic_amd/vm.py b/mimic_amd/vm.py
--- a/mimic_amd/vm.py
+++ b/mimic_amd/vm.py
@@ -860,15 +860,44 @@
 class XDPBatch:
 
     def __init__(self, pkt_data, pkt_off, pkt_len, headroom=0, tailroom=0, ingress=0, rxq=0, egress=0,
-                 schedule=L.SCHED_CHUNKED, cpu=None, step_budget=0):
+                 schedule=L.SCHED_CHUNKED, cpu=None, step_budget=0, pkt_stride=0, pkt_len_all=0, n=None,
+                 pkt_base=0):
         self.pkt_data, self.pkt_off, self.pkt_len = pkt_data, pkt_off, pkt_len
         self.headroom, self.tailroom = headroom, tailroom
         self.ingress, self.rxq, self.egress = ingress, rxq, egress
         self.schedule, self.cpu, self.step_budget = schedule, cpu, step_budget
+        self.pkt_stride, self.pkt_len_all, self.pkt_base = int(pkt_stride), int(pkt_len_all), int(pkt_base)
+        if pkt_off is not None and self.pkt_base:
+            raise ValueError("pkt_base is for batches without pkt_off")
+        if n is None:
+            if pkt_len is None and pkt_off is None:
+                raise ValueError("a batch without pkt_off and pkt_len needs an explicit n")
+            n = int((pkt_len if pkt_len is not None else pkt_off).numel())
+        self._n = int(n)
+        for a in (pkt_off, pkt_len):
+            if a is not None and int(a.numel()) != self._n:
+                raise ValueError("pkt_off / pkt_len and n disagree")
+        if not (0 <= self.pkt_stride < 1 << 32 and 0 <= self.pkt_len_all < 1 << 32):
+            raise ValueError("pkt_stride and pkt_len_all are 32-bit")
 
     @property
     def n(self) -> int:
-        return int(self.pkt_len.numel())
+        return self._n
+
+    def offset(self, i: int) -> int:
+        if self.pkt_off is None:
+            return self.pkt_base + i * self.pkt_stride
+        return int(self.pkt_off[i].item())
+
+    def length(self, i: int) -> int:
+        return self.pkt_len_all if self.pkt_len is None else int(self.pkt_len[i].item())
+
+    def offsets(self):
+        import numpy as np
+
+        if self.pkt_off is None:
+            return self.pkt_base + np.arange(self._n, dtype=np.int64) * self.pkt_stride
+        return self.pkt_off.cpu().numpy()
 
     def _c(self):
         cached = getattr(self, "_cstruct", None)
@@ -879,9 +908,11 @@
         b = L.XDPBatch()
         b.n = self.n
         b.schedule = self.schedule
-        b.pkt_data = self.pkt_data.data_ptr()
-        b.pkt_off = self.pkt_off.data_ptr()
-        b.pkt_len = self.pkt_len.data_ptr()
+        b.pkt_data = self.pkt_data.data_ptr() + (self.pkt_base if self.pkt_off is None else 0)
+        b.pkt_off = self.pkt_off.data_ptr() if self.pkt_off is not None else None
+        b.pkt_len = self.pkt_len.data_ptr() if self.pkt_len is not None else None
+        b.pkt_stride = self.pkt_stride if self.pkt_off is None else 0
+        b.pkt_len_all = self.pkt_len_all if self.pkt_len is None else 0
         b.headroom = self.headroom.data_ptr() if isinstance(self.headroom, torch.Tensor) else None
         b.headroom_all = 0 if isinstance(self.headroom, torch.Tensor) else int(self.headroom)
         b.tailroom = self.tailroom.data_ptr() if isinstance(self.tailroom, torch.Tensor) else None
@@ -951,18 +982,31 @@
         def opt(v, dt):
             return v if np.isscalar(v) else t(v, dt)
 
-        return cls(t(buf, np.uint8), t(np.asarray(off, dtype=np.uint64).view(np.int64), np.int64),
-                   t(np.asarray(lens, dtype=np.uint32).view(np.int32), np.int32),
+        off64 = np.ascontiguousarray(np.asarray(off, dtype=np.uint64))
+        len32 = np.ascontiguousarray(np.asarray(lens, dtype=np.uint32))
+        n = int(len32.shape[0])
+        compact = n > 1 and off64.shape[0] == n and os.environ.get("MIMIC_BATCH_COMPACT", "1") != "0"
+        stride = base = len_all = 0
+        drop_off = drop_len = False
+        if compact:
+            s = int(off64[1]) - int(off64[0])
+            if 0 < s < 1 << 32 and bool((off64 == off64[0] + np.arange(n, dtype=np.uint64) * np.uint64(s)).all()):
+                drop_off, stride, base = True, s, int(off64[0])
+            if bool((len32 == len32[0]).all()):
+                drop_len, len_all = True, int(len32[0])
+        return cls(t(buf, np.uint8), None if drop_off else t(off64.view(np.int64), np.int64),
+                   None if drop_len else t(len32.view(np.int32), np.int32),
                    opt(headroom, np.int32), opt(tailroom, np.int32), opt(ingress, np.int32), opt(rxq, np.int32),
-                   opt(egress, np.int32), schedule, cpu, step_budget)
+                   opt(egress, np.int32), schedule, cpu, step_budget, pkt_stride=stride, pkt_len_all=len_all, n=n,
+                   pkt_base=base)
 
     def packet_bytes(self, i: int) -> bytes:
         import numpy as np
 
-        o = int(self.pkt_off[i].item())
+        o = self.offset(i)
         h = int(self.headroom[i].item()) if not np.isscalar(self.headroom) else int(self.headroom)
         t_ = int(self.tailroom[i].item()) if not np.isscalar(self.tailroom) else int(self.tailroom)
-        n = h + int(self.pkt_len[i].item()) + t_
+        n = h + self.length(i) + t_
         return bytes(self.pkt_data[o:o + n].cpu().numpy().tobytes())
 
 
@@ -1370,7 +1414,7 @@
         cpp = [j.Context for j in js] if any(j.Context is not None for j in js) else None
         res = self.vm.RunXDPBatch(pid, batch, ctx_per_packet=cpp).numpy(len(js))
         mem = batch.pkt_data.cpu().numpy()
-        offs = batch.pkt_off.cpu().numpy()
+        offs = batch.offsets()
         for k, j in enumerate(js):
             p = j.Process
             p.Registers.R0 = int(res["r0"][k]) & 0xFFFFFFFFFFFFFFFF
```

Result: faster. 69530 Mpkts/s, median of 6 (+11.3%).
